# NVIDIA-Merlin/HugeCTR

Hardware: AMD Instinct MI355X
Metric: samples/sec (whole node) + embedding-gather HBM GB/s, DLRM Criteo-1TB (higher is better)
Workload: dtype fp16; 1 GPU; BASELINE configs[2]: DLRM Criteo-1TB slot_size_array, LocalizedSlotSparseEmbeddingHash, emb_dim=128, SGD, bs=65536 per GPU (weak scaling); batch_per_gpu=65536, global_batch=65536, slots=26, emb_dim=128, table_rows_total=187767399, parallelism=slot-sharded x1 + dp1, exchange=none (1 GPU), gather_fused_into_interaction=True

## Files before the change

### hugectr_amd/_lib.py

```python
import ctypes
import os

import torch
from ctypes import (POINTER, Structure, c_char_p, c_float, c_int, c_int64, c_size_t,
                    c_uint64, c_void_p)

_HERE = os.path.dirname(os.path.abspath(__file__))
_VARIANT = os.environ.get("HCTR_LIB_VARIANT", "")
LIB_PATH = os.path.join(_HERE, f"libhugectr_amd{'_' + _VARIANT if _VARIANT else ''}.so")

OPT_FTRL, OPT_ADAM, OPT_RMSPROP, OPT_ADAGRAD, OPT_NESTEROV, OPT_MOMENTUM_SGD, OPT_SGD = range(7)
UPDATE_LOCAL, UPDATE_GLOBAL, UPDATE_LAZY_GLOBAL = range(3)
EMB_DISTRIBUTED, EMB_LOCALIZED = 0, 1
KEY_U32, KEY_I64 = 0, 1
F32, F16, BF16 = 0, 1, 2


class EmbeddingParams(Structure):
    _fields_ = [
        ("embedding_type", c_int), ("key_type", c_int), ("out_dtype", c_int),
        ("train_batch_size", c_size_t), ("evaluate_batch_size", c_size_t),
        ("max_vocabulary_size_per_gpu", c_size_t), ("embedding_vec_size", c_size_t),
        ("max_feature_num", c_size_t), ("slot_num", c_size_t), ("combiner", c_int),
        ("slot_size_array", POINTER(c_size_t)),
# ... 44 lines not shown
    "hctr_ht_value_head": (c_int, [_P, _P, POINTER(c_size_t)]),
    "hctr_ht_set_value_head": (c_int, [_P, c_size_t, _P]),
    "hctr_ht_table_size": (c_size_t, [_P]),
    "hctr_ht_dump": (c_int, [_P, _P, _P, POINTER(c_size_t), _P]),
    "hctr_ht_error_flags": (c_int, [_P, _P, POINTER(ctypes.c_uint32)]),
    "hctr_ht_recover": (c_int, [_P, _P, c_size_t, _P]),
    "hctr_forward_pool": (c_int, [c_size_t, c_int, c_int, _P, c_int, _P, _P, _P, c_int, _P]),
    "hctr_forward_pool_weighted": (c_int, [c_size_t, c_int, c_int, _P, _P, _P, _P, _P, _P]),
    "hctr_expand_key_grads": (c_int, [c_size_t, c_int, c_int, _P, _P, _P, _P, _P]),
    "hctr_forward_pool_multihot": (c_int, [c_size_t, c_int, c_int, _P, c_int, _P, _P, _P, c_int, _P]),
    "hctr_forward_pool_mapped": (c_int, [c_size_t, c_int, c_int, _P, c_int, _P, _P, _P, c_int, c_int,
                                         c_size_t, c_size_t, _P, _P]),
    "hctr_ebc_route_whole": (c_int, [c_size_t, c_int, _P, _P, _P, c_int, _P, _P, _P, _P, c_size_t,
                                     _P]),
    "hctr_forward_reorder": (c_int, [c_size_t, c_int, c_int, c_int, _P, _P, c_int, _P]),
    "hctr_backward_reorder": (c_int, [c_size_t, c_int, c_int, c_int, _P, _P, c_int, _P]),
    "hctr_emb_create": (c_int, [POINTER(EmbeddingParams), POINTER(_P)]),
    "hctr_emb_destroy": (c_int, [_P]),
    "hctr_emb_init_params": (c_int, [_P, _P]),
    "hctr_emb_forward": (c_int, [_P, c_int, _P, _P, c_size_t, _P, _P]),
    "hctr_emb_forward_scale": (c_int, [_P, c_int, _P, _P]),
    "hctr_emb_poll_overflow": (c_int, [_P, _P]),
    "hctr_emb_backward": (c_int, [_P, _P, _P]),
    "hctr_emb_get_wgrad": (c_int, [_P, _P, _P]),
    "hctr_emb_update_params": (c_int, [_P, _P]),
    "hctr_emb_set_learning_rate": (c_int, [_P, c_float]),
    "hctr_emb_get_vocabulary_size": (c_int, [_P, _P, POINTER(c_size_t)]),
    "hctr_emb_get_max_vocabulary_size": (c_size_t, [_P]),
    "hctr_emb_slots_on_rank": (c_size_t, [_P]),
    "hctr_emb_check_overflow": (c_int, [_P, _P]),
    "hctr_emb_dump": (c_int, [_P, _P, _P, _P, POINTER(c_size_t), _P]),
    "hctr_emb_load": (c_int, [_P, _P, _P, _P, c_size_t, _P]),
    "hctr_emb_table_ptr": (_P, [_P]),
    "hctr_emb_opt_state_ptr": (_P, [_P, c_int]),
    "hctr_emb_value_index_ptr": (_P, [_P]),
    "hctr_emb_reset": (c_int, [_P, _P]),
    "hctr_emb_profiling": (c_int, [_P, c_int]),
    "hctr_emb_profile_get": (c_int, [_P, c_int, POINTER(ctypes.c_double), POINTER(c_uint64)]),
    "hctr_ebc_keys_to_indices": (c_int, [_P, c_int, c_size_t, c_int64, c_int, _P, _P]),
    "hctr_ebc_route_workspace_bytes": (c_size_t, [c_size_t, c_int]),
    "hctr_ebc_route_keys": (c_int, [c_size_t, c_int, c_int, _P, _P, _P, _P, c_int, _P, _P, _P, _P, _P]),
    "hctr_ebc_bucket_counts": (c_int, [c_size_t, c_int, c_int, c_int, _P, c_int, _P, _P]),
    "hctr_ebc_network_forward": (c_int, [c_size_t, c_int, c_int, c_int, _P, _P, _P, c_int, _P, _P, c_int, _P]),
    "hctr_ebc_network_backward": (c_int, [c_size_t, c_int, c_int, c_int, _P, _P, _P, c_int, _P, _P, c_int, _P]),
    "hctr_updater_create": (c_int, [c_size_t, c_size_t, c_int, POINTER(_P)]),
    "hctr_updater_destroy": (c_int, [_P]),
    "hctr_updater_update": (c_int, [_P, c_size_t, c_size_t, _P, _P, _P, c_int, c_int, c_int, c_float,
                                    c_float, c_float, c_float, c_float, c_float, c_uint64, _P, _P,
                                    _P, _P]),
    "hctr_interaction_fwd": (c_int, [c_size_t, c_int, c_int, _P, _P, _P, c_int, _P]),
    "hctr_interaction_bwd": (c_int, [c_size_t, c_int, c_int, _P, _P, _P, _P, _P, c_int, _P]),
    "hctr_cross_v1_fwd": (c_int, [c_size_t, c_int, c_int, _P, _P, _P, _P, _P, _P]),
    "hctr_cross_v1_bwd": (c_int, [c_size_t, c_int, c_int, _P, _P, _P, _P, _P, _P, _P, _P, _P, _P]),
    "hctr_cross_v1_bwd_workspace_bytes": (c_size_t, [c_size_t, c_int, c_int]),
    "hctr_det_create": (c_int, [c_size_t, _SZP, c_char_p, c_size_t, c_int, c_uint64, POINTER(_P)]),
    "hctr_det_destroy": (c_int, [_P]),
    "hctr_det_num_classes": (c_size_t, [_P]),
    "hctr_det_lookup": (c_int, [_P, _P, _P, c_size_t, _SZP, _SZP, c_size_t, _P]),
    "hctr_det_lookup_unsafe": (c_int, [_P, _P, _P, c_size_t, _SZP, _SZP, c_size_t, _P]),
    "hctr_det_scatter_add": (c_int, [_P, _P, _P, c_size_t, _SZP, _SZP, c_size_t, _P]),
    "hctr_det_scatter_update": (c_int, [_P, _P, _P, c_size_t, _SZP, _SZP, c_size_t, _P]),
    "hctr_det_remove": (c_int, [_P, _P, c_size_t, _SZP, _SZP, c_size_t, _P]),
    "hctr_det_export": (c_int, [_P, c_size_t, _P, _P, c_size_t, _SZP, _P]),
    "hctr_det_lookup_index": (c_int, [_P, c_size_t, _P, c_size_t, c_int, _P, _P]),
    "hctr_det_rows": (c_int, [_P, c_size_t, POINTER(_P), _SZP]),
    "hctr_det_row_store": (c_int, [_P, POINTER(_P), POINTER(ctypes.c_uint64)]),
    "hctr_det_state_store": (c_int, [_P, c_int, POINTER(_P), POINTER(_P), _P]),
    "hctr_det_lookup_rows": (c_int, [_P, _P, c_size_t, _SZP, _SZP, c_size_t, c_int, _P, _P,
                                     POINTER(c_uint64), _P]),
    "hctr_radix_sort_temp_bytes": (c_size_t, [c_size_t]),
    "hctr_radix_sort_pairs_u32": (c_int, [_P, c_size_t, _P, _P, _P, _P, c_size_t, c_int, _P]),
    "hctr_static_lookup": (c_int, [_P, c_int, c_size_t, _P, c_size_t, _P, _P, c_size_t, _P, _P, _P,
                                   _P, _P, _P, _P]),
    "hctr_forward_pool_ptrs": (c_int, [c_size_t, c_int, c_int, _P, _P, _P, c_int, _P]),
    "hctr_forward_pool_ptrs_mapped": (c_int, [c_size_t, c_int, c_int, _P, _P, _P, c_int, c_size_t,
                                              c_size_t, _P]),
    "hctr_ebc_routed_keys_to_indices": (c_int, [c_size_t, c_int, c_int, _P, _P, _P, _P, _P]),
    "hctr_ebc_local_reduce": (c_int, [_P, c_size_t, c_size_t, _P, _P, c_uint64, _P, _P, c_int, _SZP,
                                      _P, _P, _P, _P]),
    "hctr_det_clear": (c_int, [_P, _P]),
    "hctr_det_size_per_class": (c_int, [_P, _SZP, _P]),
    "hctr_det_capacity_per_class": (c_int, [_P, _SZP]),
    "hctr_det_repair_count": (c_int, [_P, POINTER(ctypes.c_uint64)]),
    "hctr_det_update": (c_int, [_P, _P, POINTER(DetOptParams), _P, c_size_t, _SZP, _SZP, c_size_t,
                                _P, _P, _P]),
    "hctr_cache_create": (c_int, [c_size_t, c_int, c_int, POINTER(_P)]),
    "hctr_cache_destroy": (c_int, [_P]),
    "hctr_cache_capacity_in_set": (c_size_t, [_P]),
    "hctr_cache_query": (c_int, [_P, _P, c_size_t, _P, _P, _P, _P, _P]),
    "hctr_cache_replace": (c_int, [_P, _P, c_size_t, _P, _P]),
    "hctr_cache_update": (c_int, [_P, _P, c_size_t, _P, _P]),
    "hctr_cache_dump": (c_int, [_P, _P, _P, c_size_t, c_size_t, _P]),
    "hctr_tiered_create": (c_int, [c_size_t, c_int, c_size_t, POINTER(_P)]),
    "hctr_tiered_destroy": (c_int, [_P]),
    "hctr_tiered_host_rows": (_P, [_P]),
    "hctr_tiered_cache": (_P, [_P]),
    "hctr_tiered_lookup": (c_int, [_P, _P, c_size_t, _P, _P, _P]),
    "hctr_tiered_scatter": (c_int, [_P, _P, c_size_t, _P, c_int, c_float, _P]),
    "hctr_tiered_flush": (c_int, [_P, _P]),
    "hctr_uvm_create": (c_int, [c_size_t, c_size_t, c_size_t, c_int, c_float, c_int, POINTER(_P)]),
    "hctr_uvm_destroy": (c_int, [_P]),
    "hctr_uvm_tier": (_P, [_P]),
    "hctr_uvm_add": (c_int, [_P, _P, _P, c_size_t]),
    "hctr_uvm_query": (c_int, [_P, _P, c_size_t, _P, _P]),
    "hctr_uvm_clear": (c_int, [_P, _P]),
    "hctr_uvm_lookup": (c_int, [_P, _P, c_size_t, _P, _P, _P, _P]),
    "hctr_uvm_scatter_rows": (c_int, [_P, _P, c_size_t, _P, c_int, c_float, _P]),
    "hctr_uvm_check_overflow": (c_int, [_P, _P]),
    "hctr_uvm_size": (c_int, [_P, _P, POINTER(c_size_t)]),
    "hctr_uniq_create": (c_int, [c_size_t, POINTER(_P)]),
    "hctr_uniq_destroy": (c_int, [_P]),
    "hctr_uniq_plan": (c_int, [_P, c_size_t, c_size_t, c_int, c_int, c_int, c_int, c_int, _P,
                               c_uint64, _P, _P, _P, _P]),
    "hctr_uniq_gather_rows": (c_int, [c_size_t, c_int, _P, _P, _P, c_int, _P]),
    "hctr_uniq_expand": (c_int, [c_size_t, c_int, _P, _P, _P, _P, c_int, c_int, _P, _P, _P, _P, _P]),
    "hctr_ebc_uniq_plan_workspace_bytes": (c_size_t, [c_size_t]),
    "hctr_ebc_uniq_plan": (c_int, [c_size_t, c_int, c_size_t, _P, _P, c_uint64, _P, _P, _P, _P,
                                   c_size_t, _P]),
    "hctr_ebc_uniq_gather_rows": (c_int, [c_size_t, c_int, _P, _P, c_uint64, _P, c_int, _P]),
    "hctr_ebc_uniq_network_forward": (c_int, [c_size_t, c_int, c_int, c_int, _P, _P, _P, c_int, _P,
                                              _P, _P, _P, _P, _P, _P, c_int, _P]),
    "hctr_ebc_uniq_backward_workspace_bytes": (c_size_t, [c_size_t, c_size_t, c_int, c_int]),
    "hctr_ebc_uniq_network_backward": (c_int, [_P, c_size_t, c_int, c_int, c_int, _P, _P, _P, _P,
                                               c_int, c_int, _P, _P, _P, c_size_t, c_size_t, _P,
                                               c_int, _P, _P, c_size_t, _P]),
    "hctr_interaction_fwd_indexed": (c_int, [c_size_t, c_int, c_int, _P, _P, _P, _P, c_int, _P]),
    "hctr_ebc_scale_average": (c_int, [c_size_t, c_int, c_int, _P, _P, c_int, _P, c_int, c_int, _P]),
    "hctr_interaction_fwd_gather": (c_int, [c_size_t, c_int, c_int, _P, _P, _P, _P, _P, c_int, _P]),
    "hctr_emb_forward_interaction": (c_int, [_P, c_int, _P, _P, _P, _P]),
    "hctr_interaction_bwd_gather": (c_int, [c_size_t, c_int, c_int, _P, _P, _P, _P, _P, _P, c_int,
                                            _P]),
    "hctr_emb_backward_interaction": (c_int, [_P, _P, _P, _P, _P, _P]),
    "hctr_interaction_bwd_indexed": (c_int, [c_size_t, c_int, c_int, _P, _P, _P, _P, _P, _P, c_int,
                                             _P]),
    "hctr_interaction_bwd_indexed_scatter": (c_int, [c_size_t, c_int, c_int, _P, _P, _P, _P, _P, _P,
                                                     c_int, _P]),
    "hctr_updater_set_ftrl": (c_int, [_P, c_float, c_float, c_float]),
    "hctr_updater_set_grad_map": (c_int, [_P, c_size_t, c_size_t]),
    "hctr_updater_set_row_bound": (c_int, [_P, ctypes.c_uint64]),
    "hctr_updater_reduce_presorted": (c_int, [_P, c_size_t, c_size_t, _P, _P, _P, _P, c_int,
                                              c_size_t, _P, _P]),
    "hctr_emb_index": (c_int, [_P, c_int, _P, _P, c_size_t, _P]),
    "hctr_emb_index_ahead": (c_int, [_P, _P, _P, c_size_t, _P]),
    "hctr_emb_index_adopt": (c_int, [_P]),
    "hctr_emb_update_rows": (c_int, [_P, c_size_t, _P, _P, _P, c_int, _P]),
    "hctr_relu_bwd_bias_workspace_bytes": (c_size_t, [c_size_t, c_int]),
    "hctr_relu_bwd_bias": (c_int, [c_size_t, c_int, _P, _P, _P, _P, _P, c_int, _P]),
    "hctr_logit_head_workspace_bytes": (c_size_t, [c_int]),
    "hctr_logit_head": (c_int, [c_size_t, c_int, _P, _P, _P, _P, c_float, _P, _P, _P, _P, _P, c_int,
                                _P]),
    "hctr_skinny_fc_fwd": (c_int, [c_size_t, c_int, c_int, _P, _P, _P, _P, c_int, _P]),
    "hctr_skinny_fc_bwd_workspace_bytes": (c_size_t, [c_int]),
    "hctr_skinny_fc_bwd": (c_int, [c_size_t, c_int, c_int, _P, _P, _P, _P, _P, _P, c_int, _P]),
    "hctr_sum_groups": (c_int, [c_int, c_size_t, _P, c_int, _P, _P]),
    "hctr_sgd_shadow": (c_int, [c_size_t, c_float, c_float, _P, _P, _P, c_int, _P]),
    "hctr_bce_loss_workspace_bytes": (c_size_t, []),
    "hctr_bce_loss": (c_int, [c_size_t, _P, _P, c_float, _P, _P, _P, c_int, _P]),
    "hctr_convert_transpose16": (c_int, [c_size_t, c_int, c_int, _P, _P, _P, c_int, _P]),
    "hctr_gemm_nt16": (c_int, [c_size_t, c_int, c_int, _P, c_int, _P, c_int, _P, c_int, c_int, _P, _P,
                               _P, _P, c_int, _P]),
    "hctr_cross_v2_bwd_step_workspace_bytes": (c_size_t, [c_size_t, c_int]),
    "hctr_cross_v2_bwd_step": (c_int, [c_size_t, c_int, _P, _P, _P, _P, _P, _P, _P, c_int, c_int, _P]),
    "hctr_lru_create": (c_int, [c_size_t, c_size_t, c_int, c_int, c_char_p, c_uint64, POINTER(_P)]),
    "hctr_lru_destroy": (c_int, [_P]),
    "hctr_lru_lookup_index": (c_int, [_P, _P, c_size_t, c_int, _P, _P, _P, _SZP, _P]),
    "hctr_lru_find": (c_int, [_P, _P, c_size_t, _P, _P]),
    "hctr_lru_rows": (c_int, [_P, POINTER(_P), _SZP]),
    "hctr_lru_state": (c_int, [_P, c_int, POINTER(_P), _P]),
    "hctr_lru_export": (c_int, [_P, _P, _P, _P, _P, c_size_t, _SZP, _P]),
    "hctr_lru_size": (c_int, [_P, _SZP, _P]),
    "hctr_lru_rejected_count": (c_int, [_P, POINTER(c_uint64), _P]),
    "hctr_lru_capacity": (c_int, [_P, _SZP, _SZP]),
    "hctr_lru_lookup_index_filtered": (c_int, [_P, _P, c_size_t, c_uint64, _P, _P, _P, _SZP, _P]),
    "hctr_lru_filtered_count": (c_int, [_P, POINTER(c_uint64), _P]),
    "hctr_lru_compact": (c_int, [_P, c_size_t, c_size_t, _P, _P, _P, _P, _P, _P, _P, _P, _SZP,
                                 _P]),
    "hctr_lru_export_if": (c_int, [_P, c_uint64, _P, _P, _P, _P, c_size_t, _SZP, _SZP, _P]),
    "hctr_lru_create_tiered": (c_int, [c_size_t, c_size_t, c_int, c_int, c_char_p, c_uint64,
                                       c_size_t, POINTER(_P)]),
    "hctr_lru_create_growing": (c_int, [c_size_t, c_size_t, c_float, c_size_t, c_int, c_int,
                                        c_char_p, c_uint64, c_size_t, POINTER(_P)]),
    "hctr_lru_growth": (c_int, [_P, _SZP, _SZP, POINTER(c_uint64)]),
    "hctr_lru_placement": (c_int, [_P, _SZP, _SZP, _SZP]),
    "hctr_lru_host_part": (c_int, [_P, c_int, POINTER(_P)]),
    "hctr_lru_gather_slots": (c_int, [_P, c_int, _P, c_size_t, _P, _P]),
    "hctr_lru_scatter_slots": (c_int, [_P, c_int, _P, c_size_t, _P, c_int, _P]),
    "hctr_lru_apply_update": (c_int, [_P, _P, c_size_t, c_size_t, _P, _P, _P, c_int, c_int,
                                      c_float, c_float, c_float, c_float, c_float, c_float,
                                      c_uint64, _P]),
    "hctr_dist_select": (c_int, [_P, c_int, c_size_t, c_int, _P, _P, _P, _P, c_size_t, _P]),
    "hctr_indexed_row_copy": (c_int, [POINTER(RowCopyTask), c_int, c_int, c_int, _P]),
    "hctr_ebc_io_create": (c_int, [c_size_t, c_int, c_int, POINTER(_P)]),
    "hctr_ebc_io_destroy": (c_int, [_P]),
    "hctr_ebc_io_chunk": (c_int, [_P, c_int, POINTER(_P), POINTER(_P), POINTER(_P), POINTER(_P)]),
    "hctr_ebc_io_wait": (c_int, [_P, c_int]),
    "hctr_ebc_io_check": (c_int, [_P, c_int, c_size_t, c_int, c_int, c_uint64, _P, _P]),
    "hctr_ebc_io_import_static": (c_int, [_P, c_int, c_size_t, c_int, c_int, c_uint64, c_uint64, _P,
                                          _P, _P, _P]),
    "hctr_ebc_io_select": (c_int, [_P, c_int, c_size_t, c_int, c_int, c_uint64, _P, _P, _P, _P, _SZP,
                                   _P]),
    "hctr_ebc_io_scatter_rows": (c_int, [c_size_t, c_int, _P, _P, _P, c_uint64, _P]),
    "hctr_ebc_io_export_static": (c_int, [_P, c_int, c_size_t, c_uint64, c_uint64, _P, _P, _P, _P]),
    "hctr_ebc_group_segments": (c_int, [c_size_t, c_size_t, _P, _P, _P, c_size_t, _P, _P]),
    "hctr_ebc_hybrid_row_ptrs": (c_int, [c_size_t, c_size_t, _P, _P, _P, c_int, _P, c_int, _P,
                                         c_size_t, _P, _P, _P]),
    "hctr_ebc_hybrid_key_grads": (c_int, [c_size_t, c_int, _P, _P, c_size_t, _P, c_int, c_size_t,
                                          c_size_t, _P, _P]),
    "hctr_metric_accumulate_temp_bytes": (c_size_t, []),
    "hctr_metric_accumulate": (c_int, [_P, c_int, _P, c_size_t, c_int, _P, _P, c_size_t, c_size_t,
                                       _P, _P, c_size_t, _P]),
    "hctr_metric_auc_temp_bytes": (c_size_t, [c_size_t]),
    "hctr_metric_auc": (c_int, [_P, c_size_t, _P, _P, c_size_t, _P, _P]),
    "hctr_metric_ndcg_temp_bytes": (c_size_t, [c_size_t]),
    "hctr_metric_ndcg": (c_int, [_P, c_size_t, _P, _P, c_size_t, _P, _P]),
}
METRIC_MAX_CLASSES = 256
METRIC_COUNTER_WORDS = 264

EXPORTED_SYMBOLS = tuple(_SIGNATURES.keys())


class HugeCTRAmdError(RuntimeError):
    """The reference surfaces C++ exceptions as Python RuntimeError; so do we."""


def _load():
    if not os.path.exists(LIB_PATH):
        raise ImportError(
            f"{LIB_PATH} not found: build it with `python -c 'import __graft_entry__ as g; "
            "g.build()'` (hipcc --offload-arch=gfx950). There is no CPU fallback.")
    lib = ctypes.CDLL(LIB_PATH)
    for name, (res, args) in _SIGNATURES.items():
        fn = getattr(lib, name)
        fn.restype = res
        fn.argtypes = args
    return lib


lib = _load()


def last_error() -> str:
    msg = lib.hctr_last_error()
    return msg.decode() if msg else ""


def check(rc: int) -> None:
    if rc != 0:
        raise HugeCTRAmdError(f"hugectr_amd error {rc}: {last_error()}")


def ptr(t):
    if t is None:
        return None
    return c_void_p(t.data_ptr())


def stream_ptr():
    import torch
    return c_void_p(torch.cuda.current_stream().cuda_stream)
```

### hugectr_amd/csrc/dense_ops.hip

```cpp
#include "block_prims.h"
#include "common.h"
#include "cvt16.h"

namespace hctr {
namespace {

typedef float f32x4 __attribute__((ext_vector_type(4)));
typedef unsigned int u32x4 __attribute__((ext_vector_type(4)));

constexpr int kBlock = 256;
constexpr int kWavesPerBlock = kBlock / 64;

__device__ __forceinline__ float wave_sum(float v) {
#pragma unroll
  for (int d = 32; d >= 1; d >>= 1) v += __shfl_xor(v, d, 64);
  return v;
}

template <int NPL>
__global__ void __launch_bounds__(kBlock)
    cross_v1_fwd_kernel(size_t batch, int w, int layers, const float* __restrict__ x0,
                        const float* __restrict__ kernels, const float* __restrict__ biases,
                        float* __restrict__ outputs, float* __restrict__ hiddens) {
  const int lane = threadIdx.x & 63;
// ... 135 lines not shown
  __shared__ float red[kBlock * 8];
  const int n8 = n / 8;
  const int c8 = threadIdx.x % cw, g = threadIdx.x / cw;
  const bool live = g < rg;
  const size_t r0 = (size_t)blockIdx.x * kRbRows;
  const size_t r1 = r0 + kRbRows < rows ? r0 + kRbRows : rows;
  for (int cc = c8; cc - c8 < n8; cc += cw) {
    float acc[8] = {0.f, 0.f, 0.f, 0.f, 0.f, 0.f, 0.f, 0.f};
    if (live && cc < n8) {
#pragma unroll 4
      for (size_t r = r0 + g; r < r1; r += rg) {
        const u32x4 gv = *reinterpret_cast<const u32x4*>(dy + r * n + cc * 8);
        const u32x4 av = *reinterpret_cast<const u32x4*>(y + r * n + cc * 8);
        u32x4 o;
#pragma unroll
        for (int e = 0; e < 4; e++) {
          const unsigned short g0 = (unsigned short)(gv[e] & 0xFFFFu);
          const unsigned short g1 = (unsigned short)(gv[e] >> 16);
          const float y0 = H::to_f32((unsigned short)(av[e] & 0xFFFFu));
          const float y1 = H::to_f32((unsigned short)(av[e] >> 16));
          const unsigned short z0 = y0 > 0.f ? g0 : (unsigned short)0;
          const unsigned short z1 = y1 > 0.f ? g1 : (unsigned short)0;
          acc[2 * e] += H::to_f32(z0);
          acc[2 * e + 1] += H::to_f32(z1);
          o[e] = (unsigned)z0 | ((unsigned)z1 << 16);
        }
        *reinterpret_cast<u32x4*>(dz + r * n + cc * 8) = o;
      }
    }
#pragma unroll
    for (int e = 0; e < 8; e++) red[e * kBlock + threadIdx.x] = acc[e];
    __syncthreads();
    if (g == 0 && cc < n8) {
      float* p = partial + (size_t)blockIdx.x * n + cc * 8;
#pragma unroll
      for (int e = 0; e < 8; e++) {
        float sum = 0.f;
        for (int k = 0; k < rg; k++) sum += red[e * kBlock + k * cw + c8];
        p[e] = sum;
      }
    }
    __syncthreads();
  }
}

template <bool BF, bool FIRST>
__global__ void __launch_bounds__(kBlock)
    cross_v2_bwd_step_kernel(size_t rows, int n, int cw, int rg, int rpt,
                             const unsigned short* __restrict__ dy,
                             const unsigned short* __restrict__ x0,
                             const unsigned short* __restrict__ hm, unsigned short* __restrict__ acc_io,
                             unsigned short* __restrict__ s0, float* __restrict__ partial) {
  using H = H16<BF>;
  __shared__ float red[kBlock * 8];
  const int n8 = n / 8;
  const int c8 = threadIdx.x % cw, g = threadIdx.x / cw;
  const bool live = g < rg;
  const size_t r0 = (size_t)blockIdx.x * (size_t)rpt;
  const size_t r1 = r0 + (size_t)rpt < rows ? r0 + (size_t)rpt : rows;
  const int cc = (int)blockIdx.y * cw + c8;
  {
    float sum[8] = {0.f, 0.f, 0.f, 0.f, 0.f, 0.f, 0.f, 0.f};
    if (live && cc < n8) {
#pragma unroll 4
      for (size_t r = r0 + g; r < r1; r += rg) {
        const size_t at = r * n + cc * 8;
        const u32x4 gv = *reinterpret_cast<const u32x4*>(dy + at);
        const u32x4 xv = *reinterpret_cast<const u32x4*>(x0 + at);
        const u32x4 hv = *reinterpret_cast<const u32x4*>(hm + at);
        u32x4 av = {0u, 0u, 0u, 0u};
        if (!FIRST) av = *reinterpret_cast<const u32x4*>(acc_io + at);
        u32x4 so, ao;
#pragma unroll
        for (int e = 0; e < 4; e++) {
          const float g0 = H::to_f32((unsigned short)(gv[e] & 0xFFFFu));
          const float g1 = H::to_f32((unsigned short)(gv[e] >> 16));
          const unsigned short p0 = H::from_f32(g0 * H::to_f32((unsigned short)(xv[e] & 0xFFFFu)));
          const unsigned short p1 = H::from_f32(g1 * H::to_f32((unsigned short)(xv[e] >> 16)));
          sum[2 * e] += H::to_f32(p0);
          sum[2 * e + 1] += H::to_f32(p1);
          so[e] = (unsigned)p0 | ((unsigned)p1 << 16);
          float a0 = g0 * H::to_f32((unsigned short)(hv[e] & 0xFFFFu));
          float a1 = g1 * H::to_f32((unsigned short)(hv[e] >> 16));
          if (!FIRST) {
            a0 += H::to_f32((unsigned short)(av[e] & 0xFFFFu));
            a1 += H::to_f32((unsigned short)(av[e] >> 16));
          }
          ao[e] = (unsigned)H::from_f32(a0) | ((unsigned)H::from_f32(a1) << 16);
        }
        *reinterpret_cast<u32x4*>(s0 + at) = so;
        *reinterpret_cast<u32x4*>(acc_io + at) = ao;
      }
    }
#pragma unroll
    for (int e = 0; e < 8; e++) red[e * kBlock + threadIdx.x] = sum[e];
    __syncthreads();
    if (g == 0 && cc < n8) {
      float* p = partial + (size_t)blockIdx.x * n + cc * 8;
#pragma unroll
      for (int e = 0; e < 8; e++) {
        float t = 0.f;
        for (int k = 0; k < rg; k++) t += red[e * kBlock + k * cw + c8];
        p[e] = t;
      }
    }
    __syncthreads();
  }
}

__global__ void __launch_bounds__(kBlock)
    colsum_partials_kernel(size_t tiles, int n, const float* __restrict__ partial,
                           float* __restrict__ db) {
  __shared__ f32x4 red[kBlock];
  const int c4 = blockIdx.x * 8 + (threadIdx.x & 7), tg = threadIdx.x >> 3;
  const bool live = c4 * 4 < n;
  f32x4 s = {0.f, 0.f, 0.f, 0.f};
  if (live) {
#pragma unroll 8
    for (size_t t = tg; t < tiles; t += 32)
      s += *reinterpret_cast<const f32x4*>(partial + t * n + c4 * 4);
  }
  red[threadIdx.x] = s;
  __syncthreads();
  if (tg == 0 && live) {
    f32x4 sum = {0.f, 0.f, 0.f, 0.f};
#pragma unroll
    for (int k = 0; k < 32; k++) sum += red[k * 8 + threadIdx.x];
    *reinterpret_cast<f32x4*>(db + c4 * 4) = sum;
  }
}

template <bool BF>
__global__ void __launch_bounds__(kBlock)
    sum_groups_kernel(int groups, size_t n8, const unsigned short* __restrict__ in,
                      float* __restrict__ out) {
  using H = H16<BF>;
  const size_t i = (size_t)blockIdx.x * kBlock + threadIdx.x;
  if (i >= n8) return;
  float acc[8] = {0.f, 0.f, 0.f, 0.f, 0.f, 0.f, 0.f, 0.f};
#pragma unroll 4
  for (int g = 0; g < groups; g++) {
    const u32x4 v = *reinterpret_cast<const u32x4*>(in + ((size_t)g * n8 + i) * 8);
#pragma unroll
    for (int e = 0; e < 4; e++) {
      acc[2 * e] += H::to_f32((unsigned short)(v[e] & 0xFFFFu));
      acc[2 * e + 1] += H::to_f32((unsigned short)(v[e] >> 16));
    }
  }
  f32x4* o = reinterpret_cast<f32x4*>(out + i * 8);
  o[0] = f32x4{acc[0], acc[1], acc[2], acc[3]};
  o[1] = f32x4{acc[4], acc[5], acc[6], acc[7]};
}

template <bool BF>
__global__ void __launch_bounds__(kBlock)
    sgd_shadow_kernel(size_t n4, float lr, float grad_scale, float* __restrict__ w,
                      const float* __restrict__ g, unsigned short* __restrict__ w16) {
  using H = H16<BF>;
  for (size_t i = (size_t)blockIdx.x * kBlock + threadIdx.x; i < n4;
       i += (size_t)gridDim.x * kBlock) {
    f32x4 wv = reinterpret_cast<f32x4*>(w)[i];
    const f32x4 gv = reinterpret_cast<const f32x4*>(g)[i];
    wv -= lr * grad_scale * gv;
    reinterpret_cast<f32x4*>(w)[i] = wv;
    const unsigned lo = (unsigned)H::from_f32(wv[0]) | ((unsigned)H::from_f32(wv[1]) << 16);
    const unsigned hi = (unsigned)H::from_f32(wv[2]) | ((unsigned)H::from_f32(wv[3]) << 16);
    reinterpret_cast<uint2*>(w16)[i] = make_uint2(lo, hi);
  }
}

constexpr int kBceBlocks = 256;

template <typename T>
__global__ void __launch_bounds__(kBlock)
    bce_kernel(size_t batch, const T* __restrict__ logit, const float* __restrict__ label,
               float grad_scale, T* __restrict__ dlogit, float* __restrict__ partial) {
  __shared__ float smem[kBlock / 64];
  float val = 0.f;
  for (size_t i = (size_t)blockIdx.x * kBlock + threadIdx.x; i < batch;
       i += (size_t)gridDim.x * kBlock) {
    const float x = ld_as_f32(logit + i);
    const float y = label[i];
    float g;
    if (x >= 0.f) {
      const float e = expf(-x);
      g = (1.f - y) - e / (1.f + e);
      val += x * (1.f - y) + logf(1.f + e);
    } else {
      const float e = expf(x);
      g = -y + e / (1.f + e);
      val += -x * y + logf(1.f + e);
    }
    if (dlogit) st_from_f32(dlogit + i, g * grad_scale);
  }
  const float tot = block_reduce_sum<float, kBlock>(val, smem);
  if (threadIdx.x == 0) partial[blockIdx.x] = tot;
}

__global__ void __launch_bounds__(kBlock)
    bce_finish_kernel(int blocks, size_t batch, const float* __restrict__ partial,
                      float* __restrict__ loss) {
  __shared__ float smem[kBlock / 64];
  const float v = (int)threadIdx.x < blocks ? partial[threadIdx.x] : 0.f;
  const float tot = block_reduce_sum<float, kBlock>(v, smem);
  if (threadIdx.x == 0) *loss = tot / (float)batch;
}

constexpr int kHeadBlocks = 1024;
constexpr int kHeadMaxSeg = 8;

template <typename T, int NSEG, int ROWS>
__global__ void __launch_bounds__(kBlock)
    logit_head_kernel(size_t batch, int K, const T* __restrict__ x, const T* __restrict__ w,
                      const T* __restrict__ bias, const float* __restrict__ label,
                      float grad_scale, T* __restrict__ dx, float* __restrict__ partial) {
  HCTR_DYN_LDS(float, lds);
  const int lane = threadIdx.x & 63, wv = threadIdx.x >> 6;
  const float4 zero4 = make_float4(0.f, 0.f, 0.f, 0.f);
  float4 wr[NSEG], acc[NSEG];
#pragma unroll
  for (int j = 0; j < NSEG; j++) {
    const int k = j * 256 + lane * 4;
    wr[j] = k < K ? ld4_as_f32<T>(w + k) : zero4;
    acc[j] = zero4;
  }
  const float b0 = ld_as_f32(bias);
  float db = 0.f, loss = 0.f;
  const size_t nw = (size_t)gridDim.x * (kBlock / 64);
  for (size_t r0 = ((size_t)blockIdx.x * (kBlock / 64) + wv) * ROWS; r0 < batch; r0 += nw * ROWS) {
    float4 xv[ROWS][NSEG];
    float dot[ROWS];
#pragma unroll
    for (int i = 0; i < ROWS; i++) {
      const size_t r = r0 + i;
      dot[i] = 0.f;
#pragma unroll
      for (int j = 0; j < NSEG; j++) {
        const int k = j * 256 + lane * 4;
        xv[i][j] = (r < batch && k < K) ? ld4_as_f32<T>(x + r * (size_t)K + k) : zero4;
        dot[i] += xv[i][j].x * wr[j].x + xv[i][j].y * wr[j].y + xv[i][j].z * wr[j].z +
                  xv[i][j].w * wr[j].w;
      }
    }
#pragma unroll
    for (int o = 32; o > 0; o >>= 1)
#pragma unroll
      for (int i = 0; i < ROWS; i++) dot[i] += __shfl_xor(dot[i], o);
#pragma unroll
    for (int i = 0; i < ROWS; i++) {
      const size_t r = r0 + i;
      if (r >= batch) break;
      const float z = dot[i] + b0;
      const float y = label[r];
      float g, l;
      if (z >= 0.f) {
        const float e = expf(-z);
        g = (1.f - y) - e / (1.f + e);
        l = z * (1.f - y) + logf(1.f + e);
      } else {
        const float e = expf(z);
        g = -y + e / (1.f + e);
        l = -z * y + logf(1.f + e);
      }
      const float dz = g * grad_scale;
      loss += l;
      db += dz;
#pragma unroll
      for (int j = 0; j < NSEG; j++) {
        const int k = j * 256 + lane * 4;
        if (k < K) {
          acc[j].x += dz * xv[i][j].x;
          acc[j].y += dz * xv[i][j].y;
          acc[j].z += dz * xv[i][j].z;
          acc[j].w += dz * xv[i][j].w;
          if (dx)
            st4_from_f32<T>(dx + r * (size_t)K + k, make_float4(dz * wr[j].x, dz * wr[j].y,
                                                                 dz * wr[j].z, dz * wr[j].w));
        }
      }
    }
  }
  float* mine = lds + wv * (K + 2);
#pragma unroll
  for (int j = 0; j < NSEG; j++) {
    const int k = j * 256 + lane * 4;
    if (k < K) {
      mine[k] = acc[j].x;
      mine[k + 1] = acc[j].y;
      mine[k + 2] = acc[j].z;
      mine[k + 3] = acc[j].w;
    }
  }
  if (lane == 0) {
    mine[K] = db;
    mine[K + 1] = loss;
  }
  __syncthreads();
  float* out = partial + (size_t)blockIdx.x * (K + 2);
  for (int k = threadIdx.x; k < K + 2; k += kBlock) {
    float t = 0.f;
    for (int q = 0; q < kBlock / 64; q++) t += lds[q * (K + 2) + k];
    out[k] = t;
  }
}

__global__ void __launch_bounds__(1024)
    logit_head_finish_kernel(int blocks, int K, size_t batch, const float* __restrict__ partial,
                             float* __restrict__ dw, float* __restrict__ db,
                             float* __restrict__ loss) {
  __shared__ float part[16][64];
  const int c = threadIdx.x & 63, grp = threadIdx.x >> 6;
  const int k = blockIdx.x * 64 + c;
  const int chunk = (blocks + 15) / 16;
  const int b0 = grp * chunk, b1 = min(blocks, b0 + chunk);
  float t = 0.f;
  if (k < K + 2) {
// ... 130 lines not shown
    }
#pragma unroll
    for (int u = 0; u < kSkinnyUnroll; u++) {
      if (r0 + (size_t)u * step < batch) {
        const float4 gf = cvt4_as_f32<T>(g[u]), af = cvt4_as_f32<T>(a[u]);
        const float d[4] = {af.x > 0.f ? gf.x : 0.f, af.y > 0.f ? gf.y : 0.f,
                            af.z > 0.f ? gf.z : 0.f, af.w > 0.f ? gf.w : 0.f};
        const float xr = lane < K ? round16<T>(xl[u]) : 0.f;
#pragma unroll
        for (int j = 0; j < 4; j++) dbv[j] += d[j];
#pragma unroll
        for (int k = 0; k < kSkinnyK; k += 2) {
          const v2f xk = v2f{__shfl(xr, k), __shfl(xr, k + 1)};
#pragma unroll
          for (int j = 0; j < 4; j++) acc[j][k / 2] += xk * d[j];
        }
      }
    }
#pragma unroll
    for (int u = 0; u < kSkinnyUnroll; u++) {
      g[u] = gn[u];
      a[u] = an[u];
      xl[u] = xn[u];
    }
  }
  const int stride = kSkinnyK + 1;
  for (int q = 0; q < kRows; q++) {
    if (sub == q && live) {
#pragma unroll
      for (int j = 0; j < 4; j++) {
        float* d = lds + (size_t)(n0 + j) * stride;
#pragma unroll
        for (int k = 0; k < kSkinnyK; k++) {
          const float v = (k & 1) ? acc[j][k / 2].y : acc[j][k / 2].x;
          d[k] = (q == 0 ? 0.f : d[k]) + v;
        }
        d[kSkinnyK] = (q == 0 ? 0.f : d[kSkinnyK]) + dbv[j];
      }
    }
    __syncthreads();
  }
  float* out = partial + (size_t)blockIdx.x * N * stride;
  for (int i = threadIdx.x; i < N * stride; i += kSkinnyBwdBlock) out[i] = lds[i];
}

typedef float v4f __attribute__((ext_vector_type(4)));
constexpr int kMfmaUnroll = 4;

template <typename T>
__global__ void __launch_bounds__(kSkinnyBwdBlock)
    skinny_fc_bwd_mfma_kernel(size_t batch, int K, int N, const float* __restrict__ x,
                              const T* __restrict__ dy, const T* __restrict__ y,
                              float* __restrict__ partial) {
  HCTR_DYN_LDS(float, lds);
  const int lane = threadIdx.x & 63;
  const int wv = __builtin_amdgcn_readfirstlane(threadIdx.x >> 6);
  constexpr int kWaves = kSkinnyBwdBlock / 64;
  const int ngroups = (N + 127) / 128;
  const int rsets = kWaves / ngroups;
  const int ng = wv % ngroups, rs = wv / ngroups;
  const bool active = rs < rsets;
  const int c = lane & 15, ri = lane >> 4;
  const int n0 = ng * 128 + 8 * c;
  const bool has_n = n0 < N;
  const int n0c = has_n ? n0 : 0;
  const int kc = c < K ? c : K - 1;
  v4f acc[8];
#pragma unroll
  for (int t = 0; t < 8; t++) acc[t] = v4f{0.f, 0.f, 0.f, 0.f};
  const size_t last = batch - 1;
  const size_t step = (size_t)gridDim.x * rsets;
  if (active) {
    for (size_t g16 = (size_t)blockIdx.x * rsets + rs; g16 * 16 < batch; g16 += step) {
      uint4 gq[kMfmaUnroll], aq[kMfmaUnroll];
      float xv[kMfmaUnroll];
#pragma unroll
      for (int u = 0; u < kMfmaUnroll; u++) {
        const size_t r = min(g16 * 16 + u * 4 + ri, last);
        gq[u] = *reinterpret_cast<const uint4*>(dy + r * (size_t)N + n0c);
        aq[u] = *reinterpret_cast<const uint4*>(y + r * (size_t)N + n0c);
        xv[u] = x[r * (size_t)K + kc];
      }
#pragma unroll
      for (int u = 0; u < kMfmaUnroll; u++) {
        const bool ok = has_n && g16 * 16 + u * 4 + ri < batch;
        const float4 g0 = cvt4_as_f32<T>(make_uint2(gq[u].x, gq[u].y));
        const float4 g1 = cvt4_as_f32<T>(make_uint2(gq[u].z, gq[u].w));
        const float4 a0 = cvt4_as_f32<T>(make_uint2(aq[u].x, aq[u].y));
        const float4 a1 = cvt4_as_f32<T>(make_uint2(aq[u].z, aq[u].w));
        const float d[8] = {(ok && a0.x > 0.f) ? g0.x : 0.f, (ok && a0.y > 0.f) ? g0.y : 0.f,
                            (ok && a0.z > 0.f) ? g0.z : 0.f, (ok && a0.w > 0.f) ? g0.w : 0.f,
                            (ok && a1.x > 0.f) ? g1.x : 0.f, (ok && a1.y > 0.f) ? g1.y : 0.f,
                            (ok && a1.z > 0.f) ? g1.z : 0.f, (ok && a1.w > 0.f) ? g1.w : 0.f};
        const float b = c < K ? round16<T>(xv[u]) : (c == K ? 1.f : 0.f);
#pragma unroll
        for (int t = 0; t < 8; t++)
          acc[t] = __builtin_amdgcn_mfma_f32_16x16x4f32(d[t], b, acc[t], 0, 0, 0);
      }
    }
  }
  const int stride = kSkinnyK + 1;
  const int col = c == K ? kSkinnyK : c;
  for (int q = 0; q < rsets; q++) {
    if (active && rs == q && c <= K) {
#pragma unroll
      for (int t = 0; t < 8; t++) {
#pragma unroll
        for (int reg = 0; reg < 4; reg++) {
          const int n = ng * 128 + 8 * (4 * ri + reg) + t;
          if (n < N) {
            float* d = lds + (size_t)n * stride + col;
            *d = (q == 0 ? 0.f : *d) + acc[t][reg];
          }
        }
      }
    }
    __syncthreads();
  }
  float* out = partial + (size_t)blockIdx.x * N * stride;
  for (int i = threadIdx.x; i < N * stride; i += kSkinnyBwdBlock) out[i] = lds[i];
}

__global__ void __launch_bounds__(1024)
    skinny_fc_finish_kernel(int blocks, int K, int N, const float* __restrict__ partial,
                            float* __restrict__ dw, float* __restrict__ db) {
  __shared__ float part[16][64];
  const int stride = kSkinnyK + 1;
  const int total = N * stride;
  const int c = threadIdx.x & 63, grp = threadIdx.x >> 6;
  const int i = blockIdx.x * 64 + c;
  const int chunk = (blocks + 15) / 16;
  const int b0 = grp * chunk, b1 = min(blocks, b0 + chunk);
  float t = 0.f;
  if (i < total) {
    int b = b0;
    for (; b + 8 <= b1; b += 8) {
      float v[8];
#pragma unroll
      for (int u = 0; u < 8; u++) v[u] = partial[(size_t)(b + u) * total + i];
#pragma unroll
      for (int u = 0; u < 8; u++) t += v[u];
    }
    for (; b < b1; b++) t += partial[(size_t)b * total + i];
  }
  part[grp][c] = t;
  __syncthreads();
  if (grp == 0 && i < total) {
    float tot = 0.f;
#pragma unroll
    for (int q = 0; q < 16; q++) tot += part[q][c];
    const int n = i / stride, k = i % stride;
    if (k == kSkinnyK) db[n] = tot;
    else if (k < K) dw[(size_t)n * K + k] = tot;
  }
}

constexpr int kCrossBwdWaves = 256 * 4;

}
}

using namespace hctr;

extern "C" {

#define HCTR_CROSS_DISPATCH(MACRO)       \
  if (npl <= 1) MACRO(1)                 \
  else if (npl <= 2) MACRO(2)            \
  else if (npl <= 4) MACRO(4)            \
  else if (npl <= 8) MACRO(8)            \
  else if (npl <= 16) MACRO(16)          \
  else if (npl <= 32) MACRO(32)          \
  else MACRO(64)

int hctr_cross_v1_fwd(size_t batch, int width, int layers, const float* x0, const float* kernels,
                      const float* biases, float* outputs, float* hiddens, hctr_stream_t stream) {
  HCTR_REQUIRE(width >= 1 && layers >= 1, "shape");
  HCTR_REQUIRE(width <= 64 * 64, "cross v1: width > 4096 not supported");
  if (batch == 0) return HCTR_OK;
  HCTR_REQUIRE(x0 && kernels && biases && outputs && hiddens, "null pointer");
  hipStream_t s = as_stream(stream);
  const int npl = (width + 63) / 64;
  const int grid = grid_for(batch * 64, kBlock);
#define HCTR_CF(N_)                                                                            \
  hipLaunchKernelGGL(cross_v1_fwd_kernel<N_>, dim3(grid), dim3(kBlock), 0, s, batch, width,    \
                     layers, x0, kernels, biases, outputs, hiddens);
  HCTR_CROSS_DISPATCH(HCTR_CF)
#undef HCTR_CF
  HCTR_LAUNCH_CHECK();
  return HCTR_OK;
}

size_t hctr_cross_v1_bwd_workspace_bytes(size_t batch, int width, int layers) {
  (void)batch;
  return (size_t)kCrossBwdWaves * layers * 2 * width * sizeof(float);
}

int hctr_cross_v1_bwd(size_t batch, int width, int layers, const float* x0, const float* kernels,
                      const float* outputs, const float* hiddens, const float* out_grad,
                      float* in_grad, float* kernel_grads, float* bias_grads, float* workspace,
                      hctr_stream_t stream) {
  HCTR_REQUIRE(width >= 1 && layers >= 1, "shape");
  HCTR_REQUIRE(width <= 64 * 64, "cross v1: width > 4096 not supported");
  HCTR_REQUIRE(x0 && kernels && outputs && hiddens && out_grad && in_grad && kernel_grads &&
                   bias_grads && workspace,
               "null pointer");
  hipStream_t s = as_stream(stream);
  const int npl = (width + 63) / 64;
  const int grid = kCrossBwdWaves / kWavesPerBlock;
  const size_t lds_bytes = (size_t)layers * 2 * width * sizeof(float);
  if (lds_bytes <= 60 * 1024) {
#define HCTR_CB(N_)                                                                           \
  hipLaunchKernelGGL((cross_v1_bwd_kernel<N_, true>), dim3(kCrossBwdWaves), dim3(64), lds_bytes, \
                     s, batch, width, layers, x0, kernels, outputs, hiddens, out_grad, in_grad,  \
                     workspace);
    HCTR_CROSS_DISPATCH(HCTR_CB)
#undef HCTR_CB
  } else {
#define HCTR_CB(N_)                                                                           \
  hipLaunchKernelGGL((cross_v1_bwd_kernel<N_, false>), dim3(grid), dim3(kBlock), 0, s, batch, \
                     width, layers, x0, kernels, outputs, hiddens, out_grad, in_grad, workspace);
    HCTR_CROSS_DISPATCH(HCTR_CB)
#undef HCTR_CB
  }
  HCTR_LAUNCH_CHECK();
  hipLaunchKernelGGL(cross_v1_reduce_kernel,
                     dim3((unsigned)ceil_div<size_t>((size_t)layers * 2 * width, 32)),
                     dim3(kBlock), 0, s, (size_t)kCrossBwdWaves, width, layers, workspace,
                     kernel_grads, bias_grads);
  HCTR_LAUNCH_CHECK();
  return HCTR_OK;
}

size_t hctr_relu_bwd_bias_workspace_bytes(size_t rows, int n) {
  return ceil_div<size_t>(rows, (size_t)kRbRows) * (size_t)n * sizeof(float);
}

int hctr_relu_bwd_bias(size_t rows, int n, const void* dy, const void* y, void* dz, float* db,
                       float* workspace, int dtype, hctr_stream_t stream) {
  HCTR_REQUIRE(n > 0 && n % 8 == 0, "n must be a multiple of 8");
  HCTR_REQUIRE(dtype == HCTR_EMB_BF16 || dtype == HCTR_EMB_F16, "16-bit dtypes only");
  if (rows == 0) return HCTR_OK;
  HCTR_REQUIRE(dy && y && dz && db && workspace, "null pointer");
  hipStream_t s = as_stream(stream);
  const size_t tiles = ceil_div<size_t>(rows, (size_t)kRbRows);
  const int cw = n / 8 < kBlock ? n / 8 : kBlock;
  const int rg = kBlock / cw;
  if (dtype == HCTR_EMB_BF16)
    hipLaunchKernelGGL(relu_bwd_bias_kernel<true>, dim3((unsigned)tiles), dim3(kBlock), 0, s, rows,
                       n, cw, rg, (const unsigned short*)dy, (const unsigned short*)y,
                       (unsigned short*)dz, workspace);
  else
    hipLaunchKernelGGL(relu_bwd_bias_kernel<false>, dim3((unsigned)tiles), dim3(kBlock), 0, s,
                       rows, n, cw, rg, (const unsigned short*)dy, (const unsigned short*)y,
                       (unsigned short*)dz, workspace);
  HCTR_LAUNCH_CHECK();
  hipLaunchKernelGGL(colsum_partials_kernel, dim3(ceil_div<int>(n, 32)), dim3(kBlock), 0, s,
                     tiles, n, workspace, db);
  HCTR_LAUNCH_CHECK();
  return HCTR_OK;
}

size_t hctr_cross_v2_bwd_step_workspace_bytes(size_t batch, int width) {
  if (batch == 0 || width <= 0) return 0;
  return ceil_div<size_t>(batch, (size_t)cross_step_rows_per_tile(batch, width)) * (size_t)width *
         sizeof(float);
}

int hctr_cross_v2_bwd_step(size_t batch, int width, const void* dy, const void* x0, const void* h,
                           void* acc, void* s0, float* db, float* workspace, int first, int dtype,
                           hctr_stream_t stream) {
  HCTR_REQUIRE(width > 0 && width % 8 == 0, "width must be a multiple of 8");
  HCTR_REQUIRE(dtype == HCTR_EMB_BF16 || dtype == HCTR_EMB_F16, "16-bit dtypes only");
  if (batch == 0) return HCTR_OK;
  HCTR_REQUIRE(dy && x0 && h && acc && s0 && db && workspace, "null pointer");
  hipStream_t s = as_stream(stream);
  const int cw = width / 8 < kBlock ? width / 8 : kBlock;
  const int rg = kBlock / cw;
  const int rpt = cross_step_rows_per_tile(batch, width);
  const size_t tiles = ceil_div<size_t>(batch, (size_t)rpt);
  const unsigned col_blocks = (unsigned)ceil_div<int>(width / 8, cw);
#define HCTR_CROSS_STEP(BF_, FIRST_)                                                              \
  hipLaunchKernelGGL((cross_v2_bwd_step_kernel<BF_, FIRST_>), dim3((unsigned)tiles, col_blocks),   \
                     dim3(kBlock), 0, s, batch, width, cw, rg, rpt, (const unsigned short*)dy,     \
                     (const unsigned short*)x0, (const unsigned short*)h, (unsigned short*)acc,    \
                     (unsigned short*)s0, workspace)
  if (dtype == HCTR_EMB_BF16) {
    if (first) HCTR_CROSS_STEP(true, true);
    else HCTR_CROSS_STEP(true, false);
  } else {
    if (first) HCTR_CROSS_STEP(false, true);
    else HCTR_CROSS_STEP(false, false);
  }
#undef HCTR_CROSS_STEP
  HCTR_LAUNCH_CHECK();
  hipLaunchKernelGGL(colsum_partials_kernel, dim3(ceil_div<int>(width, 32)), dim3(kBlock), 0, s,
                     tiles, width, workspace, db);
  HCTR_LAUNCH_CHECK();
  return HCTR_OK;
}

int hctr_sum_groups(int groups, size_t n, const void* in, int dtype, float* out,
                    hctr_stream_t stream) {
  HCTR_REQUIRE(groups > 0 && n % 8 == 0, "n must be a multiple of 8");
  HCTR_REQUIRE(dtype == HCTR_EMB_BF16 || dtype == HCTR_EMB_F16, "16-bit dtypes only");
  if (n == 0) return HCTR_OK;
  HCTR_REQUIRE(in && out, "null pointer");
  hipStream_t s = as_stream(stream);
  const size_t n8 = n / 8;
  const dim3 grid((unsigned)ceil_div<size_t>(n8, (size_t)kBlock));
  if (dtype == HCTR_EMB_BF16)
    hipLaunchKernelGGL(sum_groups_kernel<true>, grid, dim3(kBlock), 0, s, groups, n8,
                       (const unsigned short*)in, out);
  else
    hipLaunchKernelGGL(sum_groups_kernel<false>, grid, dim3(kBlock), 0, s, groups, n8,
                       (const unsigned short*)in, out);
  HCTR_LAUNCH_CHECK();
  return HCTR_OK;
}

int hctr_sgd_shadow(size_t n, float lr, float grad_scale, float* w, const float* g, void* w16,
                    int dtype, hctr_stream_t stream) {
  HCTR_REQUIRE(n % 4 == 0, "n must be a multiple of 4");
  HCTR_REQUIRE(dtype == HCTR_EMB_BF16 || dtype == HCTR_EMB_F16, "16-bit shadow dtypes only");
  if (n == 0) return HCTR_OK;
  HCTR_REQUIRE(w && g && w16, "null pointer");
  hipStream_t s = as_stream(stream);
  const dim3 grid(grid_for(n / 4, kBlock, 4096));
  if (dtype == HCTR_EMB_BF16)
    hipLaunchKernelGGL(sgd_shadow_kernel<true>, grid, dim3(kBlock), 0, s, n / 4, lr, grad_scale, w,
                       g, (unsigned short*)w16);
  else
    hipLaunchKernelGGL(sgd_shadow_kernel<false>, grid, dim3(kBlock), 0, s, n / 4, lr, grad_scale,
                       w, g, (unsigned short*)w16);
  HCTR_LAUNCH_CHECK();
  return HCTR_OK;
}

size_t hctr_bce_loss_workspace_bytes(void) { return kBceBlocks * sizeof(float); }

int hctr_bce_loss(size_t batch, const void* logit, const float* label, float grad_scale,
                  void* dlogit, float* loss, float* workspace, int dtype, hctr_stream_t stream) {
  HCTR_REQUIRE(batch > 0, "empty batch");
  HCTR_REQUIRE(logit && label && loss && workspace, "null pointer");
  hipStream_t s = as_stream(stream);
  const int blocks = (int)(ceil_div<size_t>(batch, (size_t)kBlock) < (size_t)kBceBlocks
                               ? ceil_div<size_t>(batch, (size_t)kBlock)
                               : (size_t)kBceBlocks);
  switch (dtype) {
    case HCTR_EMB_F32:
      hipLaunchKernelGGL(bce_kernel<float>, dim3(blocks), dim3(kBlock), 0, s, batch,
                         (const float*)logit, label, grad_scale, (float*)dlogit, workspace);
      break;
    case HCTR_EMB_F16:
      hipLaunchKernelGGL(bce_kernel<__half>, dim3(blocks), dim3(kBlock), 0, s, batch,
                         (const __half*)logit, label, grad_scale, (__half*)dlogit, workspace);
      break;
    case HCTR_EMB_BF16:
      hipLaunchKernelGGL(bce_kernel<__hip_bfloat16>, dim3(blocks), dim3(kBlock), 0, s, batch,
                         (const __hip_bfloat16*)logit, label, grad_scale, (__hip_bfloat16*)dlogit,
                         workspace);
      break;
    default:
      HCTR_REQUIRE(false, "bad dtype");
  }
  HCTR_LAUNCH_CHECK();
  hipLaunchKernelGGL(bce_finish_kernel, dim3(1), dim3(kBlock), 0, s, blocks, batch, workspace, loss);
  HCTR_LAUNCH_CHECK();
  return HCTR_OK;
}

size_t hctr_logit_head_workspace_bytes(int k) { return (size_t)kHeadBlocks * (k + 2) * sizeof(float); }

int hctr_logit_head(size_t batch, int k, const void* x, const void* w, const void* bias,
                    const float* label, float grad_scale, void* dx, float* dw, float* db,
                    float* loss, float* workspace, int dtype, hctr_stream_t stream) {
  HCTR_REQUIRE(batch > 0 && k >= 4 && k % 4 == 0 && k <= 256 * kHeadMaxSeg,
               "logit head: K must be a multiple of 4 and <= 2048");
  HCTR_REQUIRE(dtype == HCTR_EMB_F16 || dtype == HCTR_EMB_BF16, "16-bit activations");
  HCTR_REQUIRE(x && w && bias && label && dw && db && loss && workspace, "null pointer");
  HCTR_REQUIRE(reinterpret_cast<uintptr_t>(x) % 8 == 0 && reinterpret_cast<uintptr_t>(w) % 8 == 0 &&
                   (dx == nullptr || reinterpret_cast<uintptr_t>(dx) % 8 == 0),
               "8-byte aligned buffers");
  hipStream_t s = as_stream(stream);
  const int nseg = (k + 255) / 256;
  const int rows = nseg <= 1 ? 8 : (nseg <= 2 ? 4 : (nseg <= 4 ? 2 : 1));
  const int blocks = (int)std::min<size_t>(
      (size_t)kHeadBlocks, ceil_div<size_t>(batch, (size_t)(kBlock / 64) * rows));
  const size_t lds = (size_t)(kBlock / 64) * (k + 2) * sizeof(float);
#define HCTR_HEAD(T_, NSEG_, ROWS_)                                                               \
  hipLaunchKernelGGL((logit_head_kernel<T_, NSEG_, ROWS_>), dim3(blocks), dim3(kBlock), lds, s,   \
                     batch, k, (const T_*)x, (const T_*)w, (const T_*)bias, label, grad_scale,    \
                     (T_*)dx, workspace)
#define HCTR_HEAD_T(T_)                       \
  if (nseg <= 1) HCTR_HEAD(T_, 1, 8);         \
  else if (nseg <= 2) HCTR_HEAD(T_, 2, 4);    \
  else if (nseg <= 4) HCTR_HEAD(T_, 4, 2);    \
  else HCTR_HEAD(T_, 8, 1);
  if (dtype == HCTR_EMB_BF16) {
    HCTR_HEAD_T(__hip_bfloat16)
  } else {
    HCTR_HEAD_T(__half)
  }
#undef HCTR_HEAD_T
#undef HCTR_HEAD
  HCTR_LAUNCH_CHECK();
  hipLaunchKernelGGL(logit_head_finish_kernel, dim3(ceil_div<int>(k + 2, 64)), dim3(1024), 0, s,
                     blocks, k, batch, workspace, dw, db, loss);
  HCTR_LAUNCH_CHECK();
  return HCTR_OK;
}

static int skinny_check(size_t batch, int k, int n, int dtype) {
  HCTR_REQUIRE(batch > 0 && k >= 1 && k <= kSkinnyK, "skinny fc: 1 <= K <= 16");
  HCTR_REQUIRE(n >= 4 && n % 4 == 0 && n <= 512, "skinny fc: N a multiple of 4, <= 512");
  HCTR_REQUIRE(dtype == HCTR_EMB_F16 || dtype == HCTR_EMB_BF16, "16-bit weights / activations");
  return HCTR_OK;
}

int hctr_skinny_fc_fwd(size_t batch, int k, int n, const float* x, const void* w, const void* bias,
                       void* y, int dtype, hctr_stream_t stream) {
  HCTR_TRY(skinny_check(batch, k, n, dtype));
  HCTR_REQUIRE(x && w && bias && y, "null pointer");
  HCTR_REQUIRE(reinterpret_cast<uintptr_t>(y) % 8 == 0, "8-byte aligned output");
  hipStream_t s = as_stream(stream);
  size_t rows = ceil_div<size_t>(batch, 1024);
  rows = std::min<size_t>(256, (rows + 1) / 2 * 2);
  const int blocks = (int)ceil_div<size_t>(batch, rows);
  const size_t lds = rows * kSkinnyK * sizeof(float);
  if (dtype == HCTR_EMB_BF16)
    hipLaunchKernelGGL(skinny_fc_fwd_kernel<__hip_bfloat16>, dim3(blocks), dim3(kBlock), lds, s,
                       batch, k, n, (int)rows, x, (const __hip_bfloat16*)w,
                       (const __hip_bfloat16*)bias, (__hip_bfloat16*)y);
  else
    hipLaunchKernelGGL(skinny_fc_fwd_kernel<__half>, dim3(blocks), dim3(kBlock), lds, s, batch, k, n,
                       (int)rows, x, (const __half*)w, (const __half*)bias, (__half*)y);
  HCTR_LAUNCH_CHECK();
  return HCTR_OK;
}

size_t hctr_skinny_fc_bwd_workspace_bytes(int n) {
  return (size_t)kSkinnyBlocks * n * (kSkinnyK + 1) * sizeof(float);
}

int hctr_skinny_fc_bwd(size_t batch, int k, int n, const float* x, const void* dy, const void* y,
                       float* dw, float* db, float* workspace, int dtype, hctr_stream_t stream) {
  HCTR_TRY(skinny_check(batch, k, n, dtype));
  HCTR_REQUIRE(x && dy && y && dw && db && workspace, "null pointer");
  HCTR_REQUIRE(reinterpret_cast<uintptr_t>(dy) % 8 == 0 && reinterpret_cast<uintptr_t>(y) % 8 == 0,
               "8-byte aligned activations");
  hipStream_t s = as_stream(stream);
  const size_t lds = (size_t)n * (kSkinnyK + 1) * sizeof(float);
  const char* mode = getenv("HCTR_SKINNY_BWD");
  const bool want_mfma = mode ? strcmp(mode, "valu") != 0 : kSkinnyBwdMfmaDefault;
  if (want_mfma && k < kSkinnyK && n % 8 == 0 && reinterpret_cast<uintptr_t>(dy) % 16 == 0 &&
      reinterpret_cast<uintptr_t>(y) % 16 == 0) {
    const int rsets = (kSkinnyBwdBlock / 64) / ceil_div<int>(n, 128);
    const int blocks = (int)std::min<size_t>((size_t)kSkinnyBlocks,
                                             ceil_div<size_t>(batch, (size_t)rsets * 16));
    if (dtype == HCTR_EMB_BF16)
      hipLaunchKernelGGL(skinny_fc_bwd_mfma_kernel<__hip_bfloat16>, dim3(blocks),
                         dim3(kSkinnyBwdBlock), lds, s, batch, k, n, x, (const __hip_bfloat16*)dy,
                         (const __hip_bfloat16*)y, workspace);
    else
      hipLaunchKernelGGL(skinny_fc_bwd_mfma_kernel<__half>, dim3(blocks), dim3(kSkinnyBwdBlock), lds,
                         s, batch, k, n, x, (const __half*)dy, (const __half*)y, workspace);
    HCTR_LAUNCH_CHECK();
    hipLaunchKernelGGL(skinny_fc_finish_kernel, dim3(ceil_div<int>(n * (kSkinnyK + 1), 64)),
                       dim3(1024), 0, s, blocks, k, n, workspace, dw, db);
    HCTR_LAUNCH_CHECK();
    return HCTR_OK;
  }
  const int blocks = (int)std::min<size_t>(
      (size_t)kSkinnyBlocks, ceil_div<size_t>(batch, kSkinnyBwdBlock / kSkinnyLanes));
  if (dtype == HCTR_EMB_BF16)
    hipLaunchKernelGGL(skinny_fc_bwd_kernel<__hip_bfloat16>, dim3(blocks), dim3(kSkinnyBwdBlock), lds, s,
                       batch, k, n, x, (const __hip_bfloat16*)dy, (const __hip_bfloat16*)y,
                       workspace);
  else
    hipLaunchKernelGGL(skinny_fc_bwd_kernel<__half>, dim3(blocks), dim3(kSkinnyBwdBlock), lds, s, batch, k, n,
                       x, (const __half*)dy, (const __half*)y, workspace);
  HCTR_LAUNCH_CHECK();
  hipLaunchKernelGGL(skinny_fc_finish_kernel, dim3(ceil_div<int>(n * (kSkinnyK + 1), 64)),
                     dim3(1024), 0, s, blocks, k, n, workspace, dw, db);
  HCTR_LAUNCH_CHECK();
  return HCTR_OK;
}

}
```

### hugectr_amd/dense.py

```python
from __future__ import annotations

import os

from typing import List, Sequence

import torch

from ._lib import check, lib, ptr, stream_ptr

_DT16 = {torch.float16: 1, torch.bfloat16: 2}
_DT = {torch.float32: 0, torch.float16: 1, torch.bfloat16: 2}


def split_k_wgrad(dy: torch.Tensor, x: torch.Tensor, groups: int = 16,
                  out: torch.Tensor = None) -> torch.Tensor:
    B, o = dy.shape
    i = x.shape[1]
    g = groups
    while g > 1 and B % g != 0:
        g //= 2
    if g <= 1 or min(o, i) < 8:
        r = dy.t() @ x
        if out is not None:
            out.copy_(r)
            return out
        return r
    p = torch.bmm(dy.view(g, B // g, o).transpose(1, 2), x.view(g, B // g, i))
    if p.is_cuda and p.dtype in _DT16 and (o * i) % 8 == 0:
        if out is None:
            out = torch.empty((o, i), dtype=torch.float32, device=p.device)
        check(lib.hctr_sum_groups(g, o * i, ptr(p), _DT16[p.dtype], ptr(out), stream_ptr()))
        return out
    r = p.float().sum(0)
    if out is not None:
        out.copy_(r)
        return out
    return r


def bce_with_logits(logit: torch.Tensor, label: torch.Tensor, grad_scale: float):
    x = logit.detach().contiguous()
    y = label.contiguous()
    assert x.is_cuda and y.dtype == torch.float32 and x.numel() == y.numel()
    dlogit = torch.empty_like(x)
    loss = torch.empty(1, dtype=torch.float32, device=x.device)
    ws = torch.empty(lib.hctr_bce_loss_workspace_bytes() // 4, dtype=torch.float32, device=x.device)
    check(lib.hctr_bce_loss(x.numel(), ptr(x), ptr(y), float(grad_scale), ptr(dlogit), ptr(loss),
                            ptr(ws), _DT[x.dtype], stream_ptr()))
    return loss, dlogit


class _LinearFn(torch.autograd.Function):

    @staticmethod
    def forward(ctx, x, w_master, b_master, w16, b16, relu: bool, groups: int, gw=None, gb=None):
        x = x.contiguous()
        ctx.gw, ctx.gb = gw, gb
        if relu:
            y = torch._addmm_activation(b16, x, w16.t(), use_gelu=False)
        else:
            y = torch.addmm(b16, x, w16.t())
        ctx.relu, ctx.groups = relu, groups
        ctx.save_for_backward(x, w16, y if relu else None)
        return y

    @staticmethod
    def backward(ctx, dy):
        x, w16, y = ctx.saved_tensors
        dy = dy.contiguous()
        n = dy.shape[1]
        if ctx.relu and n % 8 == 0 and dy.dtype in _DT16 and dy.is_cuda:
            dz = torch.empty_like(dy)
            db = ctx.gb if ctx.gb is not None else torch.empty(n, dtype=torch.float32,
                                                             device=dy.device)
            ws = torch.empty(lib.hctr_relu_bwd_bias_workspace_bytes(dy.shape[0], n) // 4,
                             dtype=torch.float32, device=dy.device)
            check(lib.hctr_relu_bwd_bias(dy.shape[0], n, ptr(dy), ptr(y), ptr(dz), ptr(db), ptr(ws),
                                         _DT16[dy.dtype], stream_ptr()))
            dy = dz
        else:
            if ctx.relu:
                dy = torch.ops.aten.threshold_backward(dy, y, 0)
            db = dy.sum(0, dtype=torch.float32)
            if ctx.gb is not None:
                ctx.gb.copy_(db)
        dx = dy @ w16 if ctx.needs_input_grad[0] else None
        dw = split_k_wgrad(dy, x, ctx.groups, out=ctx.gw)
        if ctx.gw is not None:
            return dx, None, None, None, None, None, None, None, None
        return dx, dw.float(), db, None, None, None, None, None, None


class _SkinnyFirstFn(torch.autograd.Function):

    @staticmethod
    def forward(ctx, x, w_master, b_master, w16, b16, gw=None, gb=None):
        x = x.contiguous()
        B, K = x.shape
        N = w16.shape[0]
        if os.environ.get("HCTR_SKINNY_FC_FWD", "gemm") == "hip":
            y = torch.empty((B, N), dtype=w16.dtype, device=x.device)
            check(lib.hctr_skinny_fc_fwd(B, K, N, ptr(x), ptr(w16), ptr(b16), ptr(y),
                                         _DT16[w16.dtype], stream_ptr()))
        else:
            y = torch._addmm_activation(b16, x.to(w16.dtype), w16.t(), use_gelu=False)
        ctx.gw, ctx.gb = gw, gb
        ctx.save_for_backward(x, y)
        return y

    @staticmethod
    def backward(ctx, dy):
        x, y = ctx.saved_tensors
        dy = dy.contiguous()
        B, K = x.shape
        N = y.shape[1]
        dev = x.device
        dw = ctx.gw if ctx.gw is not None else torch.empty((N, K), dtype=torch.float32, device=dev)
        db = ctx.gb if ctx.gb is not None else torch.empty(N, dtype=torch.float32, device=dev)
        ws = torch.empty(lib.hctr_skinny_fc_bwd_workspace_bytes(N) // 4, dtype=torch.float32,
                         device=dev)
        check(lib.hctr_skinny_fc_bwd(B, K, N, ptr(x), ptr(dy), ptr(y), ptr(dw), ptr(db), ptr(ws),
                                     _DT16[y.dtype], stream_ptr()))
        if ctx.gw is not None:
            return None, None, None, None, None, None, None
        return None, dw, db, None, None, None, None


class _LogitHeadFn(torch.autograd.Function):

    @staticmethod
    def forward(ctx, x, w_master, b_master, w16, b16, label, grad_scale: float, gw=None, gb=None):
        x = x.contiguous()
        B, K = x.shape
        dev = x.device
        dx = torch.empty_like(x) if ctx.needs_input_grad[0] else None
        dw = gw if gw is not None else torch.empty((1, K), dtype=torch.float32, device=dev)
        db = gb if gb is not None else torch.empty(1, dtype=torch.float32, device=dev)
        loss = torch.empty(1, dtype=torch.float32, device=dev)
        ws = torch.empty(lib.hctr_logit_head_workspace_bytes(K) // 4, dtype=torch.float32, device=dev)
        label = label.contiguous()
        check(lib.hctr_logit_head(B, K, ptr(x), ptr(w16), ptr(b16), ptr(label),
                                  float(grad_scale), ptr(dx), ptr(dw), ptr(db), ptr(loss), ptr(ws),
                                  _DT16[x.dtype], stream_ptr()))
        ctx.flat = gw is not None
        ctx.dx = dx
        ctx.dw, ctx.db = (None, None) if ctx.flat else (dw, db)
        return loss

    @staticmethod
    def backward(ctx, _grad_loss):
        dx, dw, db = ctx.dx, ctx.dw, ctx.db
        ctx.dx = ctx.dw = ctx.db = None
        return dx, dw, db, None, None, None, None, None, None


class FusedMLP(torch.nn.Module):

    def __init__(self, dims: Sequence[int], last_relu: bool, dtype=torch.bfloat16,
                 wgrad_groups: int = 16):
        super().__init__()
        self.dims = list(dims)
        self.dtype = dtype
        self.wgrad_groups = wgrad_groups
        self.relu = [True] * (len(dims) - 2) + [last_relu]
        self.weights = torch.nn.ParameterList()
        self.biases = torch.nn.ParameterList()
        for i in range(len(dims) - 1):
            lin = torch.nn.Linear(dims[i], dims[i + 1])
            self.weights.append(torch.nn.Parameter(lin.weight.detach().clone()))
            self.biases.append(torch.nn.Parameter(lin.bias.detach().clone()))
        self._w16: List[torch.Tensor] = []
        self._b16: List[torch.Tensor] = []
        self.flat_w = self.flat_g = self.flat_w16 = None
        self._gw: List[torch.Tensor] = []
        self._gb: List[torch.Tensor] = []

    def flatten(self):
        dev = self.weights[0].device
        sizes = [p.numel() for p in list(self.weights) + list(self.biases)]
        offs, tot = [], 0
        for n in sizes:
            offs.append(tot)
            tot += (n + 3) // 4 * 4
        self.flat_w = torch.zeros(tot, dtype=torch.float32, device=dev)
        self.flat_g = torch.zeros(tot, dtype=torch.float32, device=dev)
        self.flat_w16 = torch.zeros(tot, dtype=self.dtype, device=dev)
        params = list(self.weights) + list(self.biases)
        views16 = []
        self._gw, self._gb = [], []
        for p, o, n in zip(params, offs, sizes):
            v = self.flat_w[o:o + n].view_as(p)
            v.copy_(p.data)
            p.data = v
            views16.append(self.flat_w16[o:o + n].view_as(p))
        nl = len(self.weights)
        self._w16, self._b16 = views16[:nl], views16[nl:]
        gviews = [self.flat_g[o:o + n].view_as(p) for p, o, n in zip(params, offs, sizes)]
        self._gw, self._gb = gviews[:nl], gviews[nl:]
        self.flat_w16.copy_(self.flat_w)
        return self

    def sgd_step(self, lr: float, grad_scale: float = 1.0):
        check(lib.hctr_sgd_shadow(self.flat_w.numel(), float(lr), float(grad_scale),
                                  ptr(self.flat_w), ptr(self.flat_g), ptr(self.flat_w16),
                                  _DT16[self.dtype], stream_ptr()))

    def refresh_shadow(self):
        if self.flat_w is not None:
            self.flat_w16.copy_(self.flat_w)
            return
        if not self._w16:
            self._w16 = [w.detach().to(self.dtype) for w in self.weights]
            self._b16 = [b.detach().to(self.dtype) for b in self.biases]
        else:
            torch._foreach_copy_(self._w16 + self._b16,
                                 [w.detach() for w in self.weights] +
                                 [b.detach() for b in self.biases])

    def _skinny_first(self, x) -> bool:
        return (self.relu[0] and self.dims[0] <= 16 and self.dims[1] % 4 == 0 and
                self.dims[1] <= 512 and self.dtype in _DT16 and x.is_cuda and
                x.dtype == torch.float32 and not x.requires_grad and
                os.environ.get("HCTR_SKINNY_FC", "1") != "0")

    def _layer(self, i, x):
        gw = self._gw[i] if self._gw else None
        gb = self._gb[i] if self._gb else None
        if i == 0 and self._skinny_first(x):
            return _SkinnyFirstFn.apply(x, self.weights[0], self.biases[0], self._w16[0],
                                        self._b16[0], gw, gb)
        if x.dtype != self.dtype:
            x = x.to(self.dtype)
        return _LinearFn.apply(x, self.weights[i], self.biases[i], self._w16[i], self._b16[i],
                               self.relu[i], self.wgrad_groups, gw, gb)

    def can_fuse_bce_head(self) -> bool:
        k = self.dims[-2]
        return (self.dims[-1] == 1 and not self.relu[-1] and k % 4 == 0 and k <= 2048 and
                self.dtype in _DT16)

    def forward_bce(self, x, label, grad_scale: float):
        assert self.can_fuse_bce_head()
        if not self._w16:
            self.refresh_shadow()
        n = len(self.weights)
        for i in range(n - 1):
            x = self._layer(i, x)
        if x.dtype != self.dtype:
            x = x.to(self.dtype)
        return _LogitHeadFn.apply(x, self.weights[-1], self.biases[-1], self._w16[-1], self._b16[-1],
                                  label, grad_scale, self._gw[-1] if self._gw else None,
                                  self._gb[-1] if self._gb else None)

    def forward(self, x):
        if not self._w16:
            self.refresh_shadow()
        for i in range(len(self.weights)):
            x = self._layer(i, x)
        return x
```

### hugectr_amd/hugectr.py

```python
from __future__ import annotations

import enum
import json
import os
import time
from dataclasses import dataclass, field
from typing import Dict, List, Optional, Sequence

import numpy as np
import torch
import torch.distributed as dist

from . import _lib
from .dense import FusedMLP, bce_with_logits
from .embedding import OptParams, SparseEmbeddingHash, backward_reorder, forward_reorder
from .embedding_collection import (DataParallelCollection, EmbeddingCollection,
                                   EmbeddingCollectionConfig, EmbeddingTableConfig)
from .metrics import EvalMetrics
from .layers import (MultiCrossLayer, interaction, interaction_gather, interaction_indexed,
                     regather_supported)
from .parallel import DistributedExchange, LocalizedExchange, reorder_row_map
from .parallel import all_reduce as _all_reduce
from . import data as _data


class Check_t(enum.Enum):
    Sum = 0
    Non = 1
    Unknown = 2


class DataReaderType_t(enum.Enum):
    Norm = 0
    Raw = 1
    Parquet = 2
    RawAsync = 3


class LrPolicy_t(enum.Enum):
    fixed = 0


class Optimizer_t(enum.IntEnum):
    Ftrl = 0
    Adam = 1
    RMSProp = 2
    AdaGrad = 3
    Nesterov = 4
    MomentumSGD = 5
    SGD = 6


class Update_t(enum.IntEnum):
    Local = 0
    Global = 1
    LazyGlobal = 2


class Embedding_t(enum.IntEnum):
    DistributedSlotSparseEmbeddingHash = 0
    LocalizedSlotSparseEmbeddingHash = 1


class Activation_t(enum.Enum):
    Relu = 0
    Non = 1
    Unspecified = 2


class Initializer_t(enum.Enum):
    Default = 0
    Uniform = 1
    XavierNorm = 2
    XavierUniform = 3
    Sinusoidal = 4
    Zero = 5


class Distribution_t(enum.Enum):
    Uniform = 0
    PowerLaw = 1


class PowerLaw_t(enum.Enum):
    Long = 0
    Medium = 1
    Short = 2
    Specific = 3


class MetricsType(enum.Enum):
    AUC = 0
    AverageLoss = 1
    HitRate = 2
    NDCG = 3
    SMAPE = 4


Layer_t = enum.Enum("Layer_t", [
    "BatchNorm", "LayerNorm", "BinaryCrossEntropyLoss", "Reshape", "Select", "Concat",
    "CrossEntropyLoss", "Dropout", "ELU", "InnerProduct", "MLP", "Interaction",
    "MultiCrossEntropyLoss", "ReLU", "ReLUHalf", "GRU", "MatrixMultiply", "MultiHeadAttention",
    "Scale", "FusedReshapeConcat", "FusedReshapeConcatGeneral", "Softmax", "PReLU_Dice",
    "ReduceMean", "Sub", "Gather", "Sigmoid", "Slice", "WeightMultiply", "FmOrder2", "Add",
    "ReduceSum", "MultiCross", "Cast", "ElementwiseMultiply", "SequenceMask", "Unknown"])


@dataclass
class Solver:
    model_name: str = ""
    seed: int = 0
    lr_policy: LrPolicy_t = LrPolicy_t.fixed
    lr: float = 0.001
    warmup_steps: int = 1
    decay_start: int = 0
    decay_steps: int = 1
    decay_power: float = 2.0
    end_lr: float = 0.0
    max_eval_batches: int = 100
    batchsize_eval: int = 2048
    batchsize: int = 2048
    vvgpu: List[List[int]] = field(default_factory=lambda: [[0]])
    repeat_dataset: bool = True
    use_mixed_precision: bool = False
    enable_tf32_compute: bool = False
    scaler: float = 1.0
    metrics_spec: Dict = field(default_factory=lambda: {MetricsType.AUC: 1.0})
    i64_input_key: bool = False
    use_algorithm_search: bool = True
    use_cuda_graph: bool = True
    gen_loss_summary: bool = True
    train_intra_iteration_overlap: bool = False
    train_inter_iteration_overlap: bool = False
    eval_intra_iteration_overlap: bool = False
    eval_inter_iteration_overlap: bool = False
    device_layout: str = "LOCAL_FIRST"
    use_embedding_collection: bool = False
    all_reduce_algo: str = "NCCL"
    grouped_all_reduce: bool = False
    num_iterations_statistics: int = 20
    perf_logging: bool = False
    drop_incomplete_batch: bool = True
    kafka_brockers: str = ""
    training_callbacks: list = field(default_factory=list)


def CreateSolver(**kw) -> Solver:
    s = Solver()
    for k, v in kw.items():
        if not hasattr(s, k):
            raise RuntimeError(f"CreateSolver: unknown argument '{k}'")
        setattr(s, k, v)
    if s.use_mixed_precision and s.scaler not in (128.0, 256.0, 512.0, 1024.0):
        raise RuntimeError("use_mixed_precision requires scaler in {128, 256, 512, 1024}")
    _launch_one_process_per_gpu(sum(len(v) for v in s.vvgpu))
    return s


def _launch_one_process_per_gpu(n_gpus: int):
    import sys
    if n_gpus <= 1 or "WORLD_SIZE" in os.environ or dist.is_initialized():
        return
    script = sys.argv[0] if sys.argv else ""
    main_file = getattr(sys.modules.get("__main__"), "__file__", None)
    direct = bool(main_file) and os.path.isfile(script) and \
        os.path.abspath(main_file) == os.path.abspath(script) and "pytest" not in sys.modules and \
        os.environ.get("HCTR_NO_RELAUNCH") != "1"
# ... 337 lines not shown
                               "launch one process per GPU (torch.distributed.run)")
        local = int(os.environ.get("LOCAL_RANK", "0"))
        if os.environ.get("HCTR_RANKS_ON_ONE_GPU") == "1":
            local = 0
        self.device = torch.device("cuda", local)
        torch.cuda.set_device(self.device)
        torch.manual_seed(solver.seed + 1)
        self.input: Optional[Input] = None
        self.embeddings: List[SparseEmbedding] = []
        self.ebc_configs: List[EmbeddingCollectionConfig] = []
        self.layers: List[DenseLayer] = []
        self._compiled = False
        self._loss = float("nan")
        self._lr = solver.lr
        self._iter = 0

    def add(self, item):
        if isinstance(item, Input):
            self.input = item
        elif isinstance(item, SparseEmbedding):
            self.embeddings.append(item)
        elif isinstance(item, EmbeddingCollectionConfig):
            self.ebc_configs.append(item)
        elif isinstance(item, DenseLayer):
            self.layers.append(item)
        else:
            raise RuntimeError(f"Model.add: unsupported item {type(item)}")

    def _emb_opt(self, se: SparseEmbedding) -> OptParams:
        o = se.optimizer if (se.optimizer is not None and se.optimizer.initialized) else self.opt
        return OptParams(optimizer=int(o.optimizer_type), update_type=int(o.update_type),
                         lr=self._lr, beta1=o.beta1, beta2=o.beta2, epsilon=o.epsilon,
                         initial_accu_value=o.initial_accu_value,
                         momentum_factor=o.momentum_factor,
                         atomic_update=bool(o.atomic_update) and
                         os.environ.get("HCTR_SGD_ATOMIC") == "1",
                         scaler=self.solver.scaler)

    def compile(self, loss_names=None, loss_weights=None):
        assert self.input is not None, "Model.add(Input(...)) first"
        self._loss_weights = dict(zip(self.input.label_names, self.input.label_weights))
        if loss_names is not None:
            ws = list(loss_weights) if loss_weights is not None else [1.0] * len(list(loss_names))
            if len(ws) != len(list(loss_names)):
                raise RuntimeError("compile: loss_names and loss_weights differ in length")
            for n, w in zip(loss_names, ws):
                if str(n) not in self.input.label_names:
                    raise RuntimeError(f"compile: '{n}' is not a label of this model "
                                       f"(labels: {self.input.label_names})")
                self._loss_weights[str(n)] = float(w)
        s = self.solver
        B, Be = s.batchsize, s.batchsize_eval
        self.bpg, self.bpg_eval = B // self.world, Be // self.world
        key_dtype = torch.int64 if s.i64_input_key else torch.uint32
        self.emb_dtype = torch.float16 if s.use_mixed_precision else torch.float32
        sp = {p.top_name: p for p in self.input.sparse_params}
        self._emb = {}
        self._shapes: Dict[str, tuple] = {self.input.dense_name: (self.input.dense_dim,)}
        for n, d in zip(self.input.label_names, self.input.label_dims):
            self._shapes[n] = (int(d),)
        for se in self.embeddings:
            p = sp[se.bottom_name]
            opt = self._emb_opt(se)
            ssa = se.slot_size_array or []
            if ssa:
                max_vocab = 0
            else:
                assert se.workspace_size_per_gpu_in_mb > 0, "workspace_size_per_gpu_in_mb or slot_size_array"
                max_vocab = _max_vocab_from_workspace(
                    se.workspace_size_per_gpu_in_mb,
                    se.optimizer if (se.optimizer is not None and se.optimizer.initialized)
                    else self.opt, se.embedding_vec_size)
            h = SparseEmbeddingHash(int(se.embedding_type), B, Be, max_vocab, se.embedding_vec_size,
                                    p.max_feature_num(), p.slot_num, se.combiner, opt,
                                    slot_size_array=ssa, key_dtype=key_dtype,
                                    out_dtype=self.emb_dtype, rank=self.rank, world=self.world,
                                    seed=s.seed, device=self.device)
            h.init_params()
            localized = se.embedding_type == Embedding_t.LocalizedSlotSparseEmbeddingHash
            ex = {}
            for mode, bb in (("train", B), ("eval", Be)):
                ex[mode] = (LocalizedExchange if localized else DistributedExchange)(
                    bb, p.slot_num, se.embedding_vec_size)
            self._emb[se.sparse_embedding_name] = (se, p, h, ex, localized)
            self._shapes[se.sparse_embedding_name] = (p.slot_num, se.embedding_vec_size)
        self._ebc = []
        for cfg in self.ebc_configs:
            subs = self._split_by_ev_size(cfg)
            if len(subs) == 1:
                subs[0][0].top_name = cfg.top_name
            for sub, ids in subs:
                rt = self._compile_ebc(sub, sp, B, Be, declare_shapes=len(subs) == 1)
                rt.update(parent=cfg, ids=ids, whole=len(subs) == 1)
                self._ebc.append(rt)
            if len(subs) > 1:
                def width(t, bottom, c):
                    h = sp[bottom].max_nnz() if str(c).lower().endswith("concat") else 1
                    return t.ev_size * max(h, 1)
                if cfg.top_name:
                    self._shapes[cfg.top_name] = (sum(width(t, b, c) for t, b, _, c in cfg.lookups),)
                else:
                    for t, b, top, c in cfg.lookups:
                        self._shapes[top] = (width(t, b, c),)
        self._mods = torch.nn.ModuleDict()
        self._loss_layer = None
        self._loss_layers = []
        for i, L in enumerate(self.layers):
            self._build_layer(i, L)
        self._mods.to(self.device)
        self._dense_params = [p for p in self._mods.parameters()]
        env = os.environ.get("HCTR_HIP_GRAPH", "auto")
        ebc_graph = bool(self.ebc_configs) and not self._emb and all(
            isinstance(rt["train"], EmbeddingCollection) for rt in self._ebc)
        self._graph_ok = (bool(s.use_cuda_graph) and env != "0" and self.world == 1 and
                          len(self._loss_layers) >= 1 and
                          ((not self.ebc_configs and len(self._loss_layers) == 1 and
                            (self.bpg <= 8192 or env == "1")) or
                           (ebc_graph and (self.bpg <= 32768 or env == "1"))))
        self._graph, self._graph_wait = None, 0
        self._dense_opt = self._make_dense_opt()
        self.reader = getattr(self, "reader_override", None) or _data.make_reader(
            self.reader_params, self.input, s, self.rank, self.world, self.device)
        self._gemm_selection = _use_gemm_selection(s)
        groups = [[p.top_name for p in rt["params"]] for rt in self._ebc]
        for j, rt in enumerate(self._ebc):
            rt["index"] = j
        for r in (getattr(self.reader, "train", None), getattr(self.reader, "evalr", None)):
            if r is not None and hasattr(r, "ebc_groups"):
                r.ebc_groups = groups
        self._plan_execution()
        self._metrics = EvalMetrics(s.metrics_spec, self.input.label_dim, self.bpg_eval,
                                    s.max_eval_batches, num_loss_layers=len(self._loss_layers),
                                    world=self.world, device=self.device)
        self._compiled = True

    def _plan_execution(self):
        s = self.solver
        consumers: Dict[str, list] = {}
        for i, L in enumerate(self.layers):
            for pos, b in enumerate(L.bottom_names):
                consumers.setdefault(b, []).append((i, pos))
        self._consumers = consumers
        fused_ok = os.environ.get("HCTR_MODEL_FUSED_DENSE", "1") != "0"
        mlps = [m for m in self._mods.values() if isinstance(m, FusedMLP)]
        in_mlps = sum(sum(q.numel() for q in m.parameters()) for m in mlps)
        total = sum(q.numel() for q in self._dense_params)
        self._flat_mlps = []
        if (fused_ok and mlps and in_mlps == total and s.use_mixed_precision and
                Optimizer_t(self.opt.optimizer_type) == Optimizer_t.SGD):
            for m in mlps:
                m.flatten()
            self._flat_mlps = mlps
            self._dense_opt = None
        self._head_layer = None
        if fused_ok and self._loss_layer is not None and s.use_mixed_precision:
            logit_name = self._loss_layer.bottom_names[0]
            for i, L in enumerate(self.layers):
                if (L.layer_type == Layer_t.MLP and L.top_names[0] == logit_name and
                        len(consumers.get(logit_name, [])) == 1 and
                        self._mods[f"l{i}"].can_fuse_bce_head()):
                    self._head_layer = i
        self._intra = bool(s.train_intra_iteration_overlap) and self.world > 1
        self._inter = bool(s.train_inter_iteration_overlap) and self.world > 1
        self._upd_overlap = bool(s.train_intra_iteration_overlap) and self.world == 1
        self._idx_mode = os.environ.get("HCTR_INDEX_AHEAD", "0")
        self._idx_overlap = (bool(s.train_inter_iteration_overlap) and self.world == 1 and
                             self._idx_mode != "0")
        want = os.environ.get("HCTR_EXCHANGE", "auto" if (self._intra and self._inter) else "rows")
        if want not in ("rows", "unique", "unique16", "auto"):
            raise RuntimeError("HCTR_EXCHANGE must be rows, unique, unique16 or auto")
        self._xstate = {}
        for name, (se, p, h, ex, localized) in self._emb.items():
            st = {"mode": "rows", "ux": None, "select": None, "indexed": False, "timing_ms": None,
                  "fused_gather": False, "rows_indexed": False}
            one_hot = p.is_fixed_length and p.max_nnz() == 1
            cons = consumers.get(name, [])
            to_interaction = (len(cons) == 1 and cons[0][1] == 1 and
                              self.layers[cons[0][0]].layer_type == Layer_t.Interaction)
            n_ins = p.slot_num + 1
            st["rows_indexed"] = (self.world > 1 and localized and to_interaction and
                                  s.use_mixed_precision and self._intra and
                                  se.embedding_vec_size in (32, 64, 128) and n_ins <= 32 and
                                  (se.embedding_vec_size + n_ins * (n_ins - 1) // 2 + 1) % 8 == 0 and
                                  os.environ.get("HCTR_ROWS_INDEXED", "1") != "0")
            if st["rows_indexed"]:
                st["row_map"] = reorder_row_map(self.bpg, p.slot_num, self.world).to(
                    self.device).contiguous()
            st["fused_gather"] = (self.world == 1 and one_hot and se.combiner == 0 and
                                  to_interaction and s.use_mixed_precision and
                                  se.embedding_vec_size in (16, 32, 64, 128) and p.slot_num <= 31 and
                                  os.environ.get("HCTR_FUSED_GATHER", "1") != "0")
            if (self.world > 1 and localized and one_hot and se.combiner == 0 and
                    want != "rows" and self._intra and
                    (se.embedding_vec_size * (2 if s.use_mixed_precision else 4)) % 16 == 0):
                try:
                    from .unique_exchange import UniqueExchange
                    st["ux"] = UniqueExchange(h, self.bpg, p.slot_num, se.embedding_vec_size)
                except Exception as e:
                    if self.rank == 0:
                        print(f"[HCTR][WARNING] unique-row exchange unavailable for {name}: {e!r}")
                if st["ux"] is not None:
                    st["indexed"] = to_interaction and s.use_mixed_precision
                    if want == "auto":
                        st["select"] = {"it": 0, "t0": 0.0, "t": {}}
                    else:
                        self._set_exchange(st, want)
            self._xstate[name] = st
        self._lookahead = None
        self._upd_stream = None
        self._idx_stream = None
        self._idx_ahead = {}
        self._upd_timing = []
        self._upd_overlap_on = True

    def _set_exchange(self, st, mode: str):
        st["mode"] = mode
        if st["ux"] is not None and mode != "rows":
            st["ux"].set_sum_dtype(self.emb_dtype if mode == "unique16" else torch.float32)

    _SEL_WARM, _SEL_TIMED, _SEL_SWITCH = 8, 3, 2

    def _select_exchange(self, st):
        sel = st["select"]
        W, T, S = self._SEL_WARM, self._SEL_TIMED, self._SEL_SWITCH
        it = sel["it"]
        sel["it"] += 1
        marks = {W: ("rows", None), W + T: ("unique", "rows"), W + T + S: ("unique", None),
                 W + 2 * T + S: (None, "unique")}
        if it not in marks:
            return
        nxt, done = marks[it]
        if done is not None or it in (W, W + T + S):
            if st["ux"] is not None:
                st["ux"].drain()
            torch.cuda.synchronize()
        if done is not None:
            sel["t"][done] = time.perf_counter() - sel["t0"]
        if it in (W, W + T + S):
            if dist.is_initialized():
                dist.barrier()
            sel["t0"] = time.perf_counter()
        if nxt is not None:
            self._set_exchange(st, nxt)
            return
        t = torch.tensor([sel["t"]["rows"], sel["t"]["unique"]], dtype=torch.float64)
        if dist.get_backend() != "gloo":
            t = t.to(self.device)
        dist.all_reduce(t, op=dist.ReduceOp.MAX)
        t = t.cpu()
        st["timing_ms"] = {"rows": float(t[0]) / T * 1e3, "unique": float(t[1]) / T * 1e3}
        self._set_exchange(st, "rows" if float(t[0]) <= float(t[1]) else "unique")
        st["select"] = None

    def exchange_report(self) -> dict:
        out = {}
        for name, (se, p, h, ex, localized) in self._emb.items():
            st = self._xstate[name]
            esz = 2 if self.solver.use_mixed_precision else 4
            D = se.embedding_vec_size
            r = {"payload": st["mode"] if self.world > 1 else "none (1 GPU)",
                 "gather_fused_into_interaction": st["fused_gather"],
                 "selection_ms_per_step": st["timing_ms"],
                 "intra_iteration_overlap": self._intra, "inter_iteration_overlap": self._inter}
            if self.world > 1 and localized and st["mode"] == "rows":
                e = ex["train"]
                r["bytes_out_forward"] = (sum(e.send) - e.send[self.rank]) * esz
                r["bytes_out_backward"] = (sum(e.recv) - e.recv[self.rank]) * esz
            elif self.world > 1 and st["ux"] is not None and st["ux"].u_send is not None:
                ux = st["ux"]
                us, ur = ux.u_send, ux.u_recv
                gsz = 2 if st["mode"] == "unique16" else 4
                r.update(distinct_rows_out=sum(us) - us[self.rank], positions=ux.P,
                         bytes_out_forward=(sum(us) - us[self.rank]) * D * esz +
                         (ux.P - ux.P // self.world) * 8,
                         bytes_out_backward=(sum(ur) - ur[self.rank]) * D * gsz)
            out[name] = r
        for i, rt in enumerate(getattr(self, "_ebc", [])):
            e = rt["train"]
            if getattr(e, "_unique", False):
                r = {"payload": "unique rows", "tables": [t.name for t in e.tables]}
                r.update(e.last_exchange or {})
                out[f"embedding_collection{i}"] = r
        return out

    def _split_by_ev_size(self, cfg: EmbeddingCollectionConfig):
        dp_names = set()
        if isinstance(cfg.shard_strategy, (list, tuple)):
            for kind, names in cfg.shard_strategy:
                if str(kind).lower() == "dp":
                    dp_names.update(str(n) for n in names)
        dp_names = {n for n in dp_names
                    if all(t.max_vocabulary_size >= 0 for t, _, _, _ in cfg.lookups if t.name == n)}
        sizes = sorted({t.ev_size for t, _, _, _ in cfg.lookups})
        comp = (getattr(cfg, "compression", None) or {}) if self.world > 1 else {}
        strategies = sorted({comp.get(t.name, "reduction") for t, _, _, _ in cfg.lookups
                             if t.name not in dp_names})
        def kind(t):
            return "hybrid" if getattr(t, "var_type", None) == "hybrid" else "plain"
        kinds = sorted({kind(t) for t, _, _, _ in cfg.lookups if t.name not in dp_names})
        if len(sizes) == 1 and not dp_names and len(strategies) <= 1 and len(kinds) <= 1:
            return [(cfg, list(range(len(cfg.lookups))))]
        tables = []
        for t, _, _, _ in cfg.lookups:
            if t not in tables:
                tables.append(t)
        own = cfg.ownership(tables, self.world)
# ... 453 lines not shown
            if localized:
                recv = ex[mode].forward(pooled)
                E = forward_reorder(recv, bpg, S, D, W) if W > 1 else pooled.view(bpg, S, D)
            else:
                E = h.forward_scale(train, ex[mode].forward(pooled).contiguous())
            if train:
                E = E.detach().requires_grad_(True)
                leaves[name] = E

                def finish(E=E):
                    g = E.grad
                    if os.environ.get("HCTR_DEBUG_LOSS_CURVE"):
                        self._last_emb_grad = g.detach().clone()
                    if localized and W > 1:
                        g = backward_reorder(g.contiguous(), bpg, S, D, W)
                    top = ex["train"].backward(g.contiguous())
                    h.backward(top.contiguous())
                    h.update_params()
                after.append(finish)
            tensors[name] = E
            return
        if st["mode"] != "rows":
            ux = st["ux"]
            ux.forward_begin(ro, keys)
            nk = nxt["sparse"][se.bottom_name] if (nxt is not None and self._inter) else None

            def resolve():
                if st["indexed"]:
                    rows, row_of = ux.forward_finish(indexed=True)
                    E = _IndexedEmb(rows, row_of, ux.backward_begin)
                else:
                    E = ux.forward_finish().detach().requires_grad_(True)
                    E.register_hook(lambda g: ux.backward_begin(g))
                if nk is not None:
                    ux.prefetch(*nk)
                return E
            tensors[name] = _Pending(resolve)
            after.append(ux.backward_finish)
            return
        pooled = h.forward(True, ro, keys)
        e = ex["train"]
        recv, work = e.forward_async(pooled)
        top_grad = torch.empty_like(pooled)
        sent = {}

        def on_grad(g):
            gsend = backward_reorder(g.contiguous(), bpg, S, D, W)
            sent["work"] = e.backward_async(gsend, top_grad.view(-1))
            sent["buf"] = gsend

        def on_rows_grad(gsend):
            sent["work"] = e.backward_async(gsend.view(-1), top_grad.view(-1))
            sent["buf"] = gsend

        def resolve():
            if work is not None:
                work.wait()
            if st["rows_indexed"]:
                return _IndexedEmb(recv.view(-1, D), st["row_map"], on_rows_grad, scatter=True)
            E = forward_reorder(recv, bpg, S, D, W).requires_grad_(True)
            E.register_hook(on_grad)
            return E

        def finish():
            if "work" not in sent:
                return
            if sent.get("work") is not None:
                sent["work"].wait()
            sent.clear()
            h.backward(top_grad)
            h.update_params()
        tensors[name] = _Pending(resolve)
        after.append(finish)

    def _ebc_tensors(self, tensors, rt, get_E):
        cfg = rt["parent"]
        span = getattr(rt["train"], "virt_span", None)

        parts = {}

        def piece(v0, reps, as_float=False):
            def resolve():
                E = get_E()
                if reps == 1:
                    if "u" not in parts:
                        parts["u"] = E.unbind(1)
                    x = parts["u"][v0]
                else:
                    x = E[:, v0:v0 + reps, :].reshape(E.shape[0], -1)
                return x.float() if as_float else x
            return _Pending(resolve)
        if rt["whole"]:
            if cfg.top_name:
                tensors[cfg.top_name] = _Pending(get_E)
            else:
                for l, (_, _, top, _) in enumerate(cfg.lookups):
                    v0, reps = span[l] if span else (l, 1)
                    tensors[top] = piece(v0, reps)
        else:
            for j, l in enumerate(rt["ids"]):
                v0, reps = span[j] if span else (j, 1)
                if cfg.top_name:
                    tensors[(id(cfg), l)] = piece(v0, reps, as_float=True)
                else:
                    tensors[cfg.lookups[l][2]] = piece(v0, reps)

    def _ebc_concat_tops(self, tensors):
        for cfg in self.ebc_configs:
            if cfg.top_name and dict.__contains__(tensors, (id(cfg), 0)):
                n = len(cfg.lookups)
                tensors[cfg.top_name] = _Pending(
                    lambda cfg=cfg, n=n: torch.cat([tensors[(id(cfg), l)] for l in range(n)], dim=1))

    def _multi_task_loss(self, tensors):
        total, probs = None, []
        for L, lg, lab in tensors["__logits__"]:
            w = self._loss_weights.get(L.bottom_names[1], 1.0)
            li = torch.nn.functional.binary_cross_entropy_with_logits(lg.float(), lab.float())
            total = li * w if total is None else total + li * w
            probs.append(torch.sigmoid(lg.float()))
        return total, probs

    def _run_batch(self, batch, train: bool, nxt=None):
        tensors = _Tensors({self.input.dense_name: batch["dense"]})
        off = 0
        for n, d in zip(self.input.label_names, self.input.label_dims):
            tensors[n] = batch["label"] if len(self.input.label_names) == 1 else \
                batch["label"][:, off:off + d]
            off += d
        leaves, after = {}, []
        for name in self._emb:
            self._emb_forward(name, batch, nxt, train, tensors, leaves, after)
        for i, rt in enumerate(self._ebc):
            self._ebc_tensors(tensors, rt, self._ebc_begin(rt, batch, train, after))
        self._ebc_concat_tops(tensors)
        label = batch["label"].float()
        gscale = self.solver.scaler / (max(self.bpg, 1) * self.world)
        head = (label, gscale) if (train and self._head_layer is not None and
                                   label.shape[1] == 1) else None
        multi = len(self._loss_layers) > 1
        if multi:
            head = None
        logit, loss = self._forward_dense(tensors, train, head)
        if multi:
            total, probs = self._multi_task_loss(tensors)
            if not train:
                return total, torch.cat(probs, dim=1)
            (total * (self.solver.scaler / self.world)).backward()
            loss = total
        elif not train:
            loss = torch.nn.functional.binary_cross_entropy_with_logits(logit, label)
            return loss, torch.sigmoid(logit)
        elif loss is not None:
            loss.backward()
        elif logit.is_cuda and label.shape == logit.shape:
            lg = tensors[self._loss_layer.bottom_names[0]]
            loss, dlogit = bce_with_logits(lg, label, gscale)
            lg.backward(dlogit)
        else:
            loss = torch.nn.functional.binary_cross_entropy_with_logits(logit, label)
            (loss * (self.solver.scaler / self.world)).backward()
        works = self._dense_reduce_begin()
        for fin in after:
            fin()
        self._dense_step(reduced=works)
        return loss.detach().reshape(()), None

    def _graph_dense(self, G, skip_step: bool):
        tensors = _Tensors({self.input.dense_name: G["dense"]})
        off = 0
        for n, d in zip(self.input.label_names, self.input.label_dims):
            tensors[n] = G["label"] if len(self.input.label_names) == 1 else \
                G["label"][:, off:off + d]
            off += d
        for name, (se, p, h, ex, localized) in self._emb.items():
            if self._xstate[name]["fused_gather"]:
                tensors[name] = _GatherEmb(h, True, lambda g, n=name: G["grads"].__setitem__(n, g))
            else:
                tensors[name] = G["leaf"][name]
        for i, rt in enumerate(self._ebc):
            self._ebc_tensors(tensors, rt, lambda i=i: G["ebc_leaf"][i])
        self._ebc_concat_tops(tensors)
        gscale = self.solver.scaler / max(self.bpg, 1)
        multi = len(self._loss_layers) > 1
        head = (G["label"], gscale) if (self._head_layer is not None and not multi and
                                        G["label"].shape[1] == 1) else None
        logit, loss = self._forward_dense(tensors, True, head)
        if multi:
            loss, _ = self._multi_task_loss(tensors)
            (loss * self.solver.scaler).backward()
        elif loss is not None:
            loss.backward()
        else:
            lg = tensors[self._loss_layer.bottom_names[0]]
            loss, dlogit = bce_with_logits(lg, G["label"], gscale)
            lg.backward(dlogit)
        for name, leaf in G["leaf"].items():
            G["grads"][name] = leaf.grad
        for i, leaf in enumerate(G["ebc_leaf"]):
            G["ebc_grads"][i] = leaf.grad
        self._dense_step(skip=skip_step)
        return loss.detach().reshape(())

    def _graph_capture(self, batch):
        B = self.bpg
        G = {"lr": self._lr, "leaf": {}, "pooled": {}, "grads": {}, "ebc_leaf": [], "ebc_grads": {},
             "dense": torch.empty_like(batch["dense"]),
             "label": torch.empty_like(batch["label"].float())}
        G["dense"].copy_(batch["dense"])
        G["label"].copy_(batch["label"].float())
        for rt in self._ebc:
            E = self._ebc_forward(rt, batch, True)
            G["ebc_leaf"].append(E.detach().clone().requires_grad_(True))
        for name, (se, p, h, ex, localized) in self._emb.items():
            ro, keys = batch["sparse"][se.bottom_name]
            if self._xstate[name]["fused_gather"]:
                h.index(True, ro, keys)
                continue
            S = h.slots_on_rank if localized else p.slot_num
            G["pooled"][name] = torch.empty((self.solver.batchsize, S, se.embedding_vec_size),
                                            dtype=self.emb_dtype, device=self.device)
            h.forward(True, ro, keys, out=G["pooled"][name])
            G["leaf"][name] = G["pooled"][name].view(B, p.slot_num, se.embedding_vec_size) \
                .requires_grad_(True)
        side = torch.cuda.Stream()
        side.wait_stream(torch.cuda.current_stream())
        with torch.cuda.stream(side):
            for _ in range(2):
                self._graph_dense(G, skip_step=True)
        torch.cuda.current_stream().wait_stream(side)
        for leaf in list(G["leaf"].values()) + G["ebc_leaf"]:
            leaf.grad = None
        for q in self._dense_params:
            q.grad = None
        G["graph"] = torch.cuda.CUDAGraph()
        with torch.cuda.graph(G["graph"]):
            G["loss"] = self._graph_dense(G, skip_step=False)
        return G

    def _graph_step(self, batch):
        G = self._graph
        fresh = G is None or G["lr"] != self._lr
        if fresh:
            G = self._graph = self._graph_capture(batch)
        else:
            for name, (se, p, h, ex, localized) in self._emb.items():
                ro, keys = batch["sparse"][se.bottom_name]
                if self._xstate[name]["fused_gather"]:
                    h.index(True, ro, keys)
                else:
                    h.forward(True, ro, keys, out=G["pooled"][name])
            for i, rt in enumerate(self._ebc):
                with torch.no_grad():
                    G["ebc_leaf"][i].copy_(self._ebc_forward(rt, batch, True))
            G["dense"].copy_(batch["dense"])
            G["label"].copy_(batch["label"])
        G["graph"].replay()
        for i, rt in enumerate(self._ebc):
            g = G["ebc_grads"].get(i)
            if g is not None:
                rt["train"].lr = self._lr
                rt["train"].backward_and_update(g.contiguous())
        for name, (se, p, h, ex, localized) in self._emb.items():
            g = G["grads"][name]
            if not self._xstate[name]["fused_gather"]:
                g = ex["train"].backward(g.contiguous())
            h.backward(g.contiguous())
            h.update_params()
        return G["loss"]

    def _dense_reduce_begin(self):
        if self.world == 1 or getattr(self, "_dense_frozen", False) or not self._intra or \
                dist.get_backend() == "gloo":
            return None
        ts = [m.flat_g for m in self._flat_mlps] if self._flat_mlps else \
            [q.grad for q in self._dense_params if q.grad is not None]
        return [dist.all_reduce(t, async_op=True) for t in ts]

    def _dense_step(self, skip: bool = False, reduced=None):
        frozen = getattr(self, "_dense_frozen", False) or skip
        if reduced is not None:
            for w in reduced:
                w.wait()
        if self._flat_mlps:
            if frozen:
                return
            for m in self._flat_mlps:
                if self.world > 1 and reduced is None:
                    _all_reduce(m.flat_g)
                m.sgd_step(self._lr, 1.0 / self.solver.scaler)
            return
        if self._dense_opt is None:
            return
        if frozen:
            self._dense_opt.zero_grad(set_to_none=True)
            return
        if self.world > 1 and reduced is None:
            for q in self._dense_params:
                if q.grad is not None:
                    _all_reduce(q.grad)
        if self.solver.scaler != 1.0:
            grads = [q.grad for q in self._dense_params if q.grad is not None]
            if grads:
                torch._foreach_div_(grads, self.solver.scaler)
        self._dense_opt.step()
        self._dense_opt.zero_grad(set_to_none=True)
        for m in self._mods.values():
            if isinstance(m, FusedMLP):
                m.refresh_shadow()

    def check_overflow(self, blocking: bool = True):
        if blocking:
            self._drain_prefetch()
        return self._check_overflow(blocking)

    def _check_overflow(self, blocking: bool = True):
        for (_, _, h, _, _) in self._emb.values():
            h.check_overflow() if blocking else h.poll_overflow()

    def train(self) -> bool:
        assert self._compiled
        for st in self._xstate.values():
            if st["select"] is not None:
                self._select_exchange(st)
        batch, self._lookahead = self._lookahead, None
        if batch is None:
            batch = self.reader.next_batch(train=True)
        if batch is None:
            return False
        nxt = None
        if (self._inter and any(st["mode"] != "rows" for st in self._xstate.values())) or \
                (self._idx_overlap and any(st["fused_gather"] for st in self._xstate.values())):
            nxt = self._lookahead = self.reader.next_batch(train=True)
        self.check_overflow(blocking=False)
        loss = None
        if self._graph_ok and not getattr(self, "_dense_frozen", False):
            if getattr(self, "_graph_lr", None) != self._lr:
                self._graph_lr, self._graph_wait, self._graph = self._lr, 3, None
            if self._graph_wait > 0:
                self._graph_wait -= 1
            else:
                try:
                    loss = self._graph_step(batch)
                except Exception as e:
                    if self._graph is not None:
                        raise
                    print(f"[HCTR][WARNING] HIP-graph capture failed ({e!r}); eager launches")
                    self._graph_ok = False
                    for q in self._dense_params:
                        q.grad = None
        if loss is None:
            loss, _ = self._run_batch(batch, True, nxt)
        self._loss_t = loss.detach()
        self._iter += 1
        return True

    def _drain_prefetch(self):
        for st in getattr(self, "_xstate", {}).values():
            if st["ux"] is not None:
                st["ux"].drain()
        for _, ev in getattr(self, "_idx_ahead", {}).values():
            torch.cuda.current_stream().wait_event(ev)

    @property
    def _eval_buf(self):
        return getattr(self, "_metrics", None)

    @_eval_buf.setter
    def _eval_buf(self, _):
        m = getattr(self, "_metrics", None)
        if m is not None:
            m.reset()

    def eval(self) -> bool:
        batch = self.reader.next_batch(train=False)
        if batch is None:
            return False
        self._drain_prefetch()
        if not self._eval_buf:
            self.check_overflow()
        with torch.no_grad():
            loss, prob = self._run_batch(batch, False)
        self._metrics.add_batch(prob, batch["label"], loss)
        return True

    def get_current_loss(self) -> float:
        return float(self._loss_t)

    def get_eval_metrics(self):
        return self._metrics.result()

    def set_learning_rate(self, lr: float):
        self._lr = lr
        for (_, _, h, _, _) in self._emb.values():
            h.set_learning_rate(lr)
        if self._dense_opt is not None:
            for g in self._dense_opt.param_groups:
                g["lr"] = lr

    def summary(self):
        if self.rank != 0:
            return
        print("=" * 67 + "Model Summary" + "=" * 67)
        print(f"{'Label':<40}{'Dense':<30}{'Sparse':<30}")
        print(f"{self.input.label_name:<40}{self.input.dense_name:<30}"
              f"{','.join(p.top_name for p in self.input.sparse_params):<30}")
        print(f"({self.bpg},{self.input.label_dim})".ljust(40) + f"({self.bpg},{self.input.dense_dim})")
        print("-" * 147)
        print(f"{'Layer Type':<40}{'Input Name':<30}{'Output Name':<30}{'Output Shape':<30}")
        for name, (se, p, h, _, _) in self._emb.items():
            print(f"{se.embedding_type.name:<40}{se.bottom_name:<30}{name:<30}"
                  f"({self.bpg},{p.slot_num},{se.embedding_vec_size})")
        for rt in self._ebc:
            cfg, e = rt["cfg"], rt["train"]
            print(f"{'EmbeddingCollection':<40}{','.join(b for _, b, _, _ in cfg.lookups)[:28]:<30}"
                  f"{(cfg.top_name or ','.join(t for _, _, t, _ in cfg.lookups))[:28]:<30}"
                  f"({self.bpg},{e.L},{e.ev})")
        for L in self.layers:
            tops = ",".join(L.top_names)
            shp = self._shapes.get(L.top_names[0], ()) if L.top_names else ()
            print(f"{L.layer_type.name:<40}{','.join(L.bottom_names):<30}{tops:<30}"
                  f"({self.bpg},{','.join(str(v) for v in shp)})")
        print("-" * 147)

    def fit(self, num_epochs=0, max_iter=2000, display=200, eval_interval=1000, snapshot=10000,
            snapshot_prefix="", data_source_params=None):
        assert self._compiled, "call compile() first"
        s = self.solver
        if self.rank == 0:
            print(f"=====================================================Model Fit====================="
                  f"================================")
            print(f"[HCTR][INFO] Use non-epoch mode with number of iterations: {max_iter}"
                  if num_epochs <= 0 else f"[HCTR][INFO] Use epoch mode with number of epochs: {num_epochs}")
            print(f"[HCTR][INFO] Training batchsize: {s.batchsize}, evaluation batchsize: {s.batchsize_eval}")
        t0 = t_fit = time.time()
        it = 0
        hit_target = False
        limit = max_iter if num_epochs <= 0 else 10 ** 12
        self._eval_buf = []
        callbacks = list(getattr(s, "training_callbacks", None) or [])
        for tc in callbacks:
# ... 420 lines not shown
```

### include/hugectr_amd.h

```cpp
#ifndef HUGECTR_AMD_H
#define HUGECTR_AMD_H
#include <stddef.h>
#include <stdint.h>

#ifdef __cplusplus
extern "C" {
#endif

typedef void* hctr_stream_t;

typedef enum {
  HCTR_OK = 0,
  HCTR_ERR_INVALID_ARG = -1,
  HCTR_ERR_HIP = -2,
  HCTR_ERR_OVERFLOW = -3,
  HCTR_ERR_UNSUPPORTED = -4,
  HCTR_ERR_IO = -5
} hctr_status;

typedef enum { HCTR_OPT_FTRL = 0, HCTR_OPT_ADAM = 1, HCTR_OPT_RMSPROP = 2, HCTR_OPT_ADAGRAD = 3,
               HCTR_OPT_NESTEROV = 4, HCTR_OPT_MOMENTUM_SGD = 5, HCTR_OPT_SGD = 6 } hctr_optimizer_t;
typedef enum { HCTR_UPDATE_LOCAL = 0, HCTR_UPDATE_GLOBAL = 1, HCTR_UPDATE_LAZY_GLOBAL = 2 } hctr_update_t;
typedef enum { HCTR_EMB_DISTRIBUTED_SLOT_HASH = 0, HCTR_EMB_LOCALIZED_SLOT_HASH = 1 } hctr_embedding_t;
typedef enum { HCTR_KEY_U32 = 0, HCTR_KEY_I64 = 1 } hctr_key_t;
// ... 190 lines not shown
int hctr_uniq_expand(size_t positions, int n_owners, const int64_t* q_off, const int64_t* r_off,
                     const uint32_t* meta, const void* rows, int vec_size, int dtype, void* out,
                     uint32_t* sorted_rows, uint32_t* sorted_buckets, uint32_t* row_of,
                     hctr_stream_t stream);
int hctr_updater_reduce_presorted(hctr_updater* u, size_t positions, size_t buckets,
                                  const int64_t* row_offset, const uint32_t* sorted_rows,
                                  const uint32_t* sorted_buckets, const void* grad, int grad_dtype,
                                  size_t n_rows, float* out_sum, hctr_stream_t stream);
size_t hctr_ebc_uniq_plan_workspace_bytes(size_t max_positions);
int hctr_ebc_uniq_plan(size_t positions, int world, size_t buckets_per_peer,
                       const int64_t* bucket_range, const uint64_t* rows, uint64_t max_row,
                       uint64_t* urow, int64_t* peer_off, uint32_t* ridx, void* workspace,
                       size_t workspace_bytes, hctr_stream_t stream);
int hctr_ebc_uniq_gather_rows(size_t n_rows, int ev_size, const uint64_t* urow, const float* table,
                              uint64_t row_bound, void* out, int out_dtype, hctr_stream_t stream);
int hctr_ebc_uniq_network_forward(size_t batch_per_gpu, int num_lookup, int ev_size, int max_shards,
                                  const int32_t* d_src_blocks, const int32_t* d_combiner,
                                  const int64_t* d_bucket_counts, int batch_major,
                                  const int64_t* recv_range, const uint32_t* ridx,
                                  const int64_t* r_off, const int32_t* d_block_source,
                                  const uint32_t* d_one_hot, const void* rows, void* out, int dtype,
                                  hctr_stream_t stream);
size_t hctr_ebc_uniq_backward_workspace_bytes(size_t max_positions, size_t batch_per_gpu,
                                              int num_lookup, int ev_size);
int hctr_ebc_uniq_network_backward(hctr_updater* u, size_t batch_per_gpu, int num_lookup,
                                   int ev_size, int num_blocks, const int32_t* d_block_lookup,
                                   const int32_t* d_block_source, const int32_t* d_combiner,
                                   const int64_t* d_bucket_counts, int batch_major, int any_average,
                                   const int64_t* recv_range, const uint32_t* ridx,
                                   const int64_t* r_off, size_t positions, size_t n_rows,
                                   const void* grad, int grad_dtype, float* out_sum,
                                   void* workspace, size_t workspace_bytes, hctr_stream_t stream);
int hctr_emb_index(hctr_embedding* emb, int is_train, const void* row_offset, const void* keys,
                   size_t nnz, hctr_stream_t stream);
int hctr_emb_index_ahead(hctr_embedding* emb, const void* row_offset, const void* keys, size_t nnz,
                         hctr_stream_t stream);
int hctr_emb_index_adopt(hctr_embedding* emb);
int hctr_emb_update_rows(hctr_embedding* emb, size_t n, const int64_t* row_offset,
                         const uint64_t* rows, const void* grad, int grad_dtype,
                         hctr_stream_t stream);

int hctr_interaction_fwd(size_t batch, int n_emb, int width, const void* mlp, const void* emb,
                         void* out, int dtype, hctr_stream_t stream);
int hctr_interaction_bwd(size_t batch, int n_emb, int width, const void* mlp, const void* emb,
                         const void* top_grad, void* mlp_grad, void* emb_grad, int dtype,
                         hctr_stream_t stream);

int hctr_interaction_fwd_indexed(size_t batch, int n_emb, int width, const void* mlp,
                                 const void* rows, const uint32_t* row_of, void* out, int dtype,
                                 hctr_stream_t stream);
int hctr_interaction_bwd_indexed(size_t batch, int n_emb, int width, const void* mlp,
                                 const void* rows, const uint32_t* row_of, const void* top_grad,
                                 void* mlp_grad, void* emb_grad, int dtype, hctr_stream_t stream);
int hctr_interaction_bwd_indexed_scatter(size_t batch, int n_emb, int width, const void* mlp,
                                         const void* rows, const uint32_t* row_of,
                                         const void* top_grad, void* mlp_grad, void* grad_rows,
                                         int dtype, hctr_stream_t stream);

int hctr_interaction_fwd_gather(size_t batch, int n_emb, int width, const void* mlp,
                                const float* table, const uint64_t* value_index, void* pooled,
                                void* out, int dtype, hctr_stream_t stream);
int hctr_interaction_bwd_gather(size_t batch, int n_emb, int width, const void* mlp,
                                const float* table, const uint64_t* value_index,
                                const void* top_grad, void* mlp_grad, void* emb_grad, int dtype,
                                hctr_stream_t stream);
int hctr_emb_forward_interaction(hctr_embedding* e, int is_train, const void* mlp, void* pooled,
                                 void* out, hctr_stream_t stream);
int hctr_emb_backward_interaction(hctr_embedding* e, const void* mlp, const void* top_grad,
                                  void* mlp_grad, void* emb_grad, hctr_stream_t stream);

int hctr_cross_v1_fwd(size_t batch, int width, int layers, const float* x0, const float* kernels,
                      const float* biases, float* outputs, float* hiddens, hctr_stream_t stream);
int hctr_cross_v1_bwd(size_t batch, int width, int layers, const float* x0, const float* kernels,
                      const float* outputs, const float* hiddens, const float* out_grad,
                      float* in_grad, float* kernel_grads, float* bias_grads, float* workspace,
                      hctr_stream_t stream);
size_t hctr_cross_v1_bwd_workspace_bytes(size_t batch, int width, int layers);

typedef struct hctr_det hctr_det;
int hctr_det_create(size_t num_classes, const size_t* dimension_per_class, const char* initializer,
                    size_t initial_capacity_per_class, int key_type, uint64_t seed,
                    hctr_det** out);
int hctr_det_destroy(hctr_det* h);
size_t hctr_det_num_classes(const hctr_det* h);
int hctr_det_lookup(hctr_det* h, const void* keys, float* elements, size_t num_keys,
                    const size_t* id_spaces, const size_t* id_space_offsets, size_t num_id_spaces,
                    hctr_stream_t stream);
int hctr_det_lookup_unsafe(hctr_det* h, const void* keys, float** elements, size_t num_keys,
                           const size_t* id_spaces, const size_t* id_space_offsets,
                           size_t num_id_spaces, hctr_stream_t stream);
int hctr_det_scatter_add(hctr_det* h, const void* keys, const float* elements, size_t num_keys,
                         const size_t* id_spaces, const size_t* id_space_offsets,
                         size_t num_id_spaces, hctr_stream_t stream);
int hctr_det_scatter_update(hctr_det* h, const void* keys, const float* elements, size_t num_keys,
                            const size_t* id_spaces, const size_t* id_space_offsets,
                            size_t num_id_spaces, hctr_stream_t stream);
int hctr_det_remove(hctr_det* h, const void* keys, size_t num_keys, const size_t* id_spaces,
                    const size_t* id_space_offsets, size_t num_id_spaces, hctr_stream_t stream);
int hctr_det_export(hctr_det* h, size_t class_index, void* keys, float* values, size_t num_keys,
                    size_t* exported, hctr_stream_t stream);
int hctr_det_lookup_index(hctr_det* h, size_t class_index, const void* keys, size_t num_keys,
                          int insert, uint64_t* row_index, hctr_stream_t stream);
int hctr_det_rows(hctr_det* h, size_t class_index, float** rows, size_t* capacity);
int hctr_det_row_store(hctr_det* h, float** rows, uint64_t* total_rows);
int hctr_det_state_store(hctr_det* h, int num_state, float** state0, float** state1,
                         hctr_stream_t stream);
int hctr_det_lookup_rows(hctr_det* h, const void* keys, size_t num_keys, const size_t* id_spaces,
                         const size_t* id_space_offsets, size_t num_id_spaces, int insert,
                         float** elements, uint64_t* row_index, uint64_t* class_row_base,
                         hctr_stream_t stream);
int hctr_det_clear(hctr_det* h, hctr_stream_t stream);
int hctr_det_size_per_class(hctr_det* h, size_t* sizes, hctr_stream_t stream);
int hctr_det_capacity_per_class(const hctr_det* h, size_t* capacities);
int hctr_det_repair_count(const hctr_det* h, uint64_t* out);

typedef struct {
  int optimizer;
  float lr, beta1, beta2, epsilon;
  float momentum_factor;
  float rmsprop_beta;
  float ftrl_lambda1, ftrl_lambda2, ftrl_beta;
  float scaler;
} hctr_det_opt_params;
int hctr_det_update(hctr_det* weights, hctr_det* states, const hctr_det_opt_params* p,
                    const void* unique_keys, size_t num_unique_keys, const size_t* id_spaces,
                    const size_t* id_space_offsets, size_t num_id_spaces,
                    const uint32_t* ev_start_indices, const float* wgrad, hctr_stream_t stream);

size_t hctr_relu_bwd_bias_workspace_bytes(size_t rows, int n);
int hctr_relu_bwd_bias(size_t rows, int n, const void* dy, const void* y, void* dz, float* db,
                       float* workspace, int dtype, hctr_stream_t stream);

int hctr_sum_groups(int groups, size_t n, const void* in, int dtype, float* out,
                    hctr_stream_t stream);

int hctr_sgd_shadow(size_t n, float lr, float grad_scale, float* w, const float* g, void* w16,
                    int dtype, hctr_stream_t stream);

size_t hctr_bce_loss_workspace_bytes(void);
int hctr_bce_loss(size_t batch, const void* logit, const float* label, float grad_scale,
                  void* dlogit, float* loss, float* workspace, int dtype, hctr_stream_t stream);

size_t hctr_logit_head_workspace_bytes(int k);
int hctr_logit_head(size_t batch, int k, const void* x, const void* w, const void* bias,
                    const float* label, float grad_scale, void* dx, float* dw, float* db,
                    float* loss, float* workspace, int dtype, hctr_stream_t stream);

int hctr_skinny_fc_fwd(size_t batch, int k, int n, const float* x, const void* w, const void* bias,
                       void* y, int dtype, hctr_stream_t stream);
size_t hctr_skinny_fc_bwd_workspace_bytes(int n);
int hctr_skinny_fc_bwd(size_t batch, int k, int n, const float* x, const void* dy, const void* y,
                       float* dw, float* db, float* workspace, int dtype, hctr_stream_t stream);

int hctr_gemm_nt16(size_t m, int n, int k, const void* a, int lda, const void* bt, int ldb, void* c,
                   int ldc, int epilogue, const void* bias, const void* x0, const void* xl,
                   void* h_out, int dtype, hctr_stream_t stream);
int hctr_convert_transpose16(size_t batch, int rows, int cols, const float* src, void* dst,
                             void* dst_t, int dtype, hctr_stream_t stream);
size_t hctr_cross_v2_bwd_step_workspace_bytes(size_t batch, int width);
int hctr_cross_v2_bwd_step(size_t batch, int width, const void* dy, const void* x0, const void* h,
                           void* acc, void* s0, float* db, float* workspace, int first, int dtype,
                           hctr_stream_t stream);

typedef struct hctr_cache hctr_cache;
int hctr_cache_create(size_t capacity_in_set, int vec_size, int key_type, hctr_cache** out);
int hctr_cache_destroy(hctr_cache* c);
size_t hctr_cache_capacity_in_set(const hctr_cache* c);
int hctr_cache_query(hctr_cache* c, const void* keys, size_t len, float* values,
                     uint64_t* missing_index, void* missing_keys, size_t* d_missing_len,
                     hctr_stream_t stream);
int hctr_cache_replace(hctr_cache* c, const void* keys, size_t len, const float* values,
                       hctr_stream_t stream);
int hctr_cache_update(hctr_cache* c, const void* keys, size_t len, const float* values,
                      hctr_stream_t stream);
int hctr_cache_dump(hctr_cache* c, void* keys, size_t* d_dump_counter, size_t start_set_index,
                    size_t end_set_index, hctr_stream_t stream);

typedef struct hctr_tiered hctr_tiered;
int hctr_tiered_create(size_t host_rows, int vec_size, size_t cache_capacity_in_set,
                       hctr_tiered** out);
int hctr_tiered_destroy(hctr_tiered* t);
float* hctr_tiered_host_rows(hctr_tiered* t);
hctr_cache* hctr_tiered_cache(hctr_tiered* t);
int hctr_tiered_lookup(hctr_tiered* t, const int64_t* keys, size_t len, float* out,
                       size_t* d_missing_len, hctr_stream_t stream);
int hctr_tiered_scatter(hctr_tiered* t, const int64_t* unique_keys, size_t len, const float* values,
                        int add, float alpha, hctr_stream_t stream);
int hctr_tiered_flush(hctr_tiered* t, hctr_stream_t stream);

typedef struct hctr_uvm hctr_uvm;
int hctr_uvm_create(size_t device_table_capacity, size_t host_table_capacity, size_t max_batch_size,
                    int vec_size, float default_value, int key_type, hctr_uvm** out);
int hctr_uvm_destroy(hctr_uvm* u);
hctr_tiered* hctr_uvm_tier(hctr_uvm* u);
int hctr_uvm_add(hctr_uvm* u, const void* h_keys, const float* h_vectors, size_t len);
int hctr_uvm_query(hctr_uvm* u, const void* d_keys, size_t len, float* d_vectors,
                   hctr_stream_t stream);
int hctr_uvm_clear(hctr_uvm* u, hctr_stream_t stream);
int hctr_uvm_lookup(hctr_uvm* u, const void* d_keys, size_t len, float* d_vectors,
                    uint64_t* d_row_index, size_t* d_missing_len, hctr_stream_t stream);
int hctr_uvm_scatter_rows(hctr_uvm* u, const uint64_t* d_unique_rows, size_t len,
                          const float* values, int add, float alpha, hctr_stream_t stream);
int hctr_uvm_check_overflow(hctr_uvm* u, hctr_stream_t stream);
int hctr_uvm_size(hctr_uvm* u, hctr_stream_t stream, size_t* out);

typedef struct hctr_lru hctr_lru;
int hctr_lru_create(size_t capacity, size_t bucket_size, int dim, int key_type,
                    const char* initializer, uint64_t seed, hctr_lru** out);
int hctr_lru_destroy(hctr_lru* h);
int hctr_lru_lookup_index(hctr_lru* h, const void* keys, size_t n, int insert, uint64_t* row_index,
                          void* evict_keys, float* evict_rows, size_t* n_evicted,
                          hctr_stream_t stream);
int hctr_lru_find(hctr_lru* h, const void* keys, size_t n, uint64_t* row_index,
                  hctr_stream_t stream);
int hctr_lru_rows(hctr_lru* h, float** rows, size_t* capacity);
int hctr_lru_state(hctr_lru* h, int i, float** state, hctr_stream_t stream);
int hctr_lru_export(hctr_lru* h, void* keys, uint64_t* slots, uint64_t* scores, float* rows,
                    size_t max_keys, size_t* exported, hctr_stream_t stream);
int hctr_lru_size(hctr_lru* h, size_t* out, hctr_stream_t stream);
int hctr_lru_rejected_count(hctr_lru* h, uint64_t* out, hctr_stream_t stream);
int hctr_lru_capacity(const hctr_lru* h, size_t* capacity, size_t* bucket_size);
#define HCTR_LRU_FILTERED 0xFFFFFFFFFFFFFFFEull
int hctr_lru_lookup_index_filtered(hctr_lru* h, const void* keys, size_t n, uint64_t admit_below,
                                   uint64_t* row_index, void* evict_keys, float* evict_rows,
                                   size_t* n_evicted, hctr_stream_t stream);
int hctr_lru_filtered_count(hctr_lru* h, uint64_t* out, hctr_stream_t stream);
int hctr_lru_compact(hctr_lru* h, size_t batch, size_t n, const long long* offsets,
                     const uint64_t* rows, const void* keys, const float* weights,
                     long long* out_offsets, uint64_t* out_rows, void* out_keys,
                     float* out_weights, size_t* n_kept, hctr_stream_t stream);
int hctr_lru_export_if(hctr_lru* h, uint64_t min_score, void* keys, uint64_t* slots,
                       uint64_t* scores, float* rows, size_t max_keys, size_t* exported,
                       size_t* matched, hctr_stream_t stream);
int hctr_lru_create_tiered(size_t capacity, size_t bucket_size, int dim, int key_type,
                           const char* initializer, uint64_t seed, size_t hbm_slots,
                           hctr_lru** out);
int hctr_lru_placement(const hctr_lru* h, size_t* hbm_slots, size_t* hbm_rows, size_t* host_rows);
int hctr_lru_host_part(const hctr_lru* h, int array, float** host);
int hctr_lru_gather_slots(hctr_lru* h, int array, const uint64_t* slots, size_t n, float* out,
                          hctr_stream_t stream);
int hctr_lru_scatter_slots(hctr_lru* h, int array, const uint64_t* slots, size_t n,
                           const float* values, int add, hctr_stream_t stream);
int hctr_lru_apply_update(hctr_lru* h, hctr_updater* u, size_t buckets, size_t nnz,
                          const int64_t* bucket_range, const uint64_t* slots, const void* grad,
                          int grad_dtype, int optimizer, float lr, float beta1, float beta2,
                          float epsilon, float momentum_factor, float scaler, uint64_t times,
                          hctr_stream_t stream);
int hctr_lru_create_growing(size_t init_capacity, size_t max_capacity, float max_load_factor,
                            size_t bucket_size, int dim, int key_type, const char* initializer,
                            uint64_t seed, size_t hbm_slots, hctr_lru** out);
int hctr_lru_growth(const hctr_lru* h, size_t* capacity_now, size_t* capacity_max,
                    uint64_t* doublings);


#define HCTR_DIST_SELECT_WS_BYTES(num_splits) ((size_t)8 * ((size_t)(num_splits) * 1024 + 1))
int hctr_dist_select(const void* keys, int key_type, size_t n, int num_splits, void* out_keys,
                     int32_t* order, int32_t* splits, void* workspace, size_t workspace_bytes,
                     hctr_stream_t stream);

#define HCTR_ROW_COPY_MAX_TASKS 32
typedef struct {
  const void* src;
  size_t src_rows;
  int dim;
  int index_type;
  const void* index;
  uint64_t index_div;
  size_t n;
  void* dst;
  size_t dst_rows;
  const int32_t* dst_pos;
} hctr_row_copy_task;
int hctr_indexed_row_copy(const hctr_row_copy_task* tasks, int num_tasks, int src_dtype,
                          int dst_dtype, hctr_stream_t stream);

typedef struct hctr_ebc_io hctr_ebc_io;
int hctr_ebc_io_create(size_t chunk_rows, int ev_size, int key_type, hctr_ebc_io** out);
int hctr_ebc_io_destroy(hctr_ebc_io* io);
int hctr_ebc_io_chunk(hctr_ebc_io* io, int which, void** keys, float** rows, float** state0,
                      float** state1);
int hctr_ebc_io_wait(hctr_ebc_io* io, int which);
int hctr_ebc_io_check(hctr_ebc_io* io, int which, size_t n, int num_shards, int shard_id,
                      uint64_t vocab, uint64_t* d_counts, hctr_stream_t stream);
int hctr_ebc_io_import_static(hctr_ebc_io* io, int which, size_t n, int num_shards, int shard_id,
                              uint64_t vocab, uint64_t row_start, float* table, float* state0,
                              float* state1, hctr_stream_t stream);
int hctr_ebc_io_select(hctr_ebc_io* io, int which, size_t n, int num_shards, int shard_id,
                       uint64_t vocab, int64_t* out_keys, float* out_rows, float* out_state0,
                       float* out_state1, size_t* selected, hctr_stream_t stream);
int hctr_ebc_io_scatter_rows(size_t n, int ev_size, const uint64_t* row_index, const float* src,
                             float* dst, uint64_t row_bound, hctr_stream_t stream);
int hctr_ebc_io_export_static(hctr_ebc_io* io, int which, size_t n, uint64_t first_key,
                              uint64_t key_step, const float* table_rows, const float* state0,
                              const float* state1, hctr_stream_t stream);

int hctr_ebc_group_segments(size_t n_seg, size_t seg_stride, const int64_t* seg_offsets,
                            const int64_t* seg_dst, const int64_t* keys, size_t nnz,
                            int64_t* out_keys, hctr_stream_t stream);
int hctr_ebc_hybrid_row_ptrs(size_t n_seg, size_t seg_stride, const int64_t* seg_offsets,
                             const int64_t* seg_dst, const int32_t* seg_table, int n_tables,
                             const uint64_t* table_desc, int ev_size, const uint64_t* rows,
                             size_t nnz, const float** out_ptrs, uint32_t* out_perm,
                             hctr_stream_t stream);
int hctr_ebc_hybrid_key_grads(size_t buckets, int ev_size, const int64_t* bucket_range,
                              const uint32_t* perm, size_t nnz, const void* grad, int grad_dtype,
                              size_t samples, size_t lookups, float* key_grads,
// ... 21 lines not shown
```

Measured before the change: 30.45 million samples/s.

## Fuse dense gradient reductions and SGD update into one segmented finish kernel

The per-layer gradient finishing kernels (group sums, bias column sums, logit-head and skinny-FC partial reductions) are deferred and merged into a single segmented kernel driven by a device-side segment table. On one GPU that kernel also applies SGD and writes the fp16/bf16 shadow weights directly, so the separate gradient write and sgd_shadow pass go away. The goal is fewer kernel launches and less memory traffic over the dense gradients in each step, paid for with a table rebuild whenever the segment layout changes and a more complex code path. The loss backward also reuses a cached ones tensor instead of allocating one every step.

```diff
diff --git a/hugectr_amd/_lib.py b/hugectr_amd/_lib.py
--- a/hugectr_amd/_lib.py
+++ b/hugectr_amd/_lib.py
@@ -220,6 +220,14 @@
     "hctr_skinny_fc_fwd": (c_int, [c_size_t, c_int, c_int, _P, _P, _P, _P, c_int, _P]),
     "hctr_skinny_fc_bwd_workspace_bytes": (c_size_t, [c_int]),
     "hctr_skinny_fc_bwd": (c_int, [c_size_t, c_int, c_int, _P, _P, _P, _P, _P, _P, c_int, _P]),
+    "hctr_relu_bwd_bias_partials": (c_int, [c_size_t, c_int, _P, _P, _P, _P, c_int, _P]),
+    "hctr_logit_head_blocks": (c_int, [c_size_t, c_int]),
+    "hctr_logit_head_partials": (c_int, [c_size_t, c_int, _P, _P, _P, _P, c_float, _P, _P, c_int,
+                                         _P]),
+    "hctr_skinny_fc_bwd_blocks": (c_int, [c_size_t, c_int, c_int, _P, _P]),
+    "hctr_skinny_fc_bwd_partials": (c_int, [c_size_t, c_int, c_int, _P, _P, _P, _P, c_int, _P]),
+    "hctr_dense_seg_blocks": (c_int, [c_int, c_size_t]),
+    "hctr_dense_grad_finish": (c_int, [_P, c_int, c_size_t, c_int, c_float, c_float, _P, _P]),
     "hctr_sum_groups": (c_int, [c_int, c_size_t, _P, c_int, _P, _P]),
     "hctr_sgd_shadow": (c_int, [c_size_t, c_float, c_float, _P, _P, _P, c_int, _P]),
     "hctr_bce_loss_workspace_bytes": (c_size_t, []),
diff --git a/hugectr_amd/csrc/dense_ops.hip b/hugectr_amd/csrc/dense_ops.hip
--- a/hugectr_amd/csrc/dense_ops.hip
+++ b/hugectr_amd/csrc/dense_ops.hip
@@ -311,6 +311,12 @@
   o[1] = f32x4{acc[4], acc[5], acc[6], acc[7]};
 }
 
+template <typename V>
+__device__ __forceinline__ V sgd_apply(V w, V g, float lr, float grad_scale) {
+  w -= lr * grad_scale * g;
+  return w;
+}
+
 template <bool BF>
 __global__ void __launch_bounds__(kBlock)
     sgd_shadow_kernel(size_t n4, float lr, float grad_scale, float* __restrict__ w,
@@ -320,7 +326,7 @@
        i += (size_t)gridDim.x * kBlock) {
     f32x4 wv = reinterpret_cast<f32x4*>(w)[i];
     const f32x4 gv = reinterpret_cast<const f32x4*>(g)[i];
-    wv -= lr * grad_scale * gv;
+    wv = sgd_apply(wv, gv, lr, grad_scale);
     reinterpret_cast<f32x4*>(w)[i] = wv;
     const unsigned lo = (unsigned)H::from_f32(wv[0]) | ((unsigned)H::from_f32(wv[1]) << 16);
     const unsigned hi = (unsigned)H::from_f32(wv[2]) | ((unsigned)H::from_f32(wv[3]) << 16);
@@ -757,6 +763,179 @@
     const int n = i / stride, k = i % stride;
     if (k == kSkinnyK) db[n] = tot;
     else if (k < K) dw[(size_t)n * K + k] = tot;
+  }
+}
+
+template <bool SGD>
+__device__ __forceinline__ void finish_store4(const hctr_dense_seg& sg, size_t at, f32x4 gv,
+                                              float lr, float grad_scale) {
+  if (!SGD) {
+    *reinterpret_cast<f32x4*>(reinterpret_cast<float*>(sg.g) + at) = gv;
+    return;
+  }
+  f32x4* wp = reinterpret_cast<f32x4*>(reinterpret_cast<float*>(sg.w) + at);
+  const f32x4 wv = sgd_apply(*wp, gv, lr, grad_scale);
+  *wp = wv;
+  unsigned lo, hi;
+  if (sg.bf16) {
+    lo = (unsigned)H16<true>::from_f32(wv[0]) | ((unsigned)H16<true>::from_f32(wv[1]) << 16);
+    hi = (unsigned)H16<true>::from_f32(wv[2]) | ((unsigned)H16<true>::from_f32(wv[3]) << 16);
+  } else {
+    lo = (unsigned)H16<false>::from_f32(wv[0]) | ((unsigned)H16<false>::from_f32(wv[1]) << 16);
+    hi = (unsigned)H16<false>::from_f32(wv[2]) | ((unsigned)H16<false>::from_f32(wv[3]) << 16);
+  }
+  *reinterpret_cast<uint2*>(reinterpret_cast<unsigned short*>(sg.w16) + at) = make_uint2(lo, hi);
+}
+
+template <bool SGD>
+__device__ __forceinline__ void finish_store1(const hctr_dense_seg& sg, size_t at, float gv,
+                                              float lr, float grad_scale) {
+  if (!SGD) {
+    reinterpret_cast<float*>(sg.g)[at] = gv;
+    return;
+  }
+  float* wp = reinterpret_cast<float*>(sg.w) + at;
+  const float wv = sgd_apply(*wp, gv, lr, grad_scale);
+  *wp = wv;
+  reinterpret_cast<unsigned short*>(sg.w16)[at] =
+      sg.bf16 ? H16<true>::from_f32(wv) : H16<false>::from_f32(wv);
+}
+
+template <bool BF>
+__device__ __forceinline__ void finish_sum_groups(int groups, size_t n8, size_t i,
+                                                  const unsigned short* __restrict__ in,
+                                                  f32x4& lo, f32x4& hi) {
+  using H = H16<BF>;
+  float acc[8] = {0.f, 0.f, 0.f, 0.f, 0.f, 0.f, 0.f, 0.f};
+#pragma unroll 16
+  for (int g = 0; g < groups; g++) {
+    const u32x4 v = *reinterpret_cast<const u32x4*>(in + ((size_t)g * n8 + i) * 8);
+#pragma unroll
+    for (int e = 0; e < 4; e++) {
+      acc[2 * e] += H::to_f32((unsigned short)(v[e] & 0xFFFFu));
+      acc[2 * e + 1] += H::to_f32((unsigned short)(v[e] >> 16));
+    }
+  }
+  lo = f32x4{acc[0], acc[1], acc[2], acc[3]};
+  hi = f32x4{acc[4], acc[5], acc[6], acc[7]};
+}
+
+__device__ __forceinline__ float finish_block_chunks(float (*part)[64], int blocks, size_t stride,
+                                                     size_t col, bool live,
+                                                     const float* __restrict__ partial) {
+  const int c = threadIdx.x & 63;
+  const int chunk = (blocks + 15) / 16;
+  for (int grp = threadIdx.x >> 6; grp < 16; grp += kBlock / 64) {
+    const int b0 = grp * chunk, b1 = min(blocks, b0 + chunk);
+    float t = 0.f;
+    if (live) {
+      int b = b0;
+      for (; b + 8 <= b1; b += 8) {
+        float v[8];
+#pragma unroll
+        for (int u = 0; u < 8; u++) v[u] = partial[(size_t)(b + u) * stride + col];
+#pragma unroll
+        for (int u = 0; u < 8; u++) t += v[u];
+      }
+      for (; b < b1; b++) t += partial[(size_t)b * stride + col];
+    }
+    part[grp][c] = t;
+  }
+  __syncthreads();
+  float tot = 0.f;
+  if (threadIdx.x < 64 && live) {
+#pragma unroll
+    for (int g = 0; g < 16; g++) tot += part[g][c];
+  }
+  return tot;
+}
+
+template <bool SGD>
+__global__ void __launch_bounds__(kBlock)
+    dense_grad_finish_kernel(const hctr_dense_seg* __restrict__ segs, int nseg, float lr,
+                             float grad_scale, float* __restrict__ loss) {
+  __shared__ f32x4 red[kBlock];
+  int si = -1;
+  for (int base = 0; base < nseg; base += 64) {
+    const int t = base + (int)(threadIdx.x & 63);
+    const bool in = t < nseg && segs[t].block0 <= (long long)blockIdx.x;
+    si += (int)__popcll(__ballot(in));
+  }
+  const hctr_dense_seg sg = segs[si];
+  const int blk = (int)((long long)blockIdx.x - sg.block0);
+  const size_t dst = (size_t)sg.dst, dst2 = (size_t)sg.dst2;
+  switch ((int)sg.kind) {
+    case HCTR_DENSE_SEG_SUM_GROUPS: {
+      const size_t n8 = (size_t)sg.n / 8;
+      const size_t i = (size_t)blk * kBlock + threadIdx.x;
+      if (i >= n8) return;
+      const unsigned short* in = reinterpret_cast<const unsigned short*>(sg.src);
+      f32x4 lo, hi;
+      if (sg.src_bf16) finish_sum_groups<true>((int)sg.count, n8, i, in, lo, hi);
+      else finish_sum_groups<false>((int)sg.count, n8, i, in, lo, hi);
+      finish_store4<SGD>(sg, dst + i * 8, lo, lr, grad_scale);
+      finish_store4<SGD>(sg, dst + i * 8 + 4, hi, lr, grad_scale);
+      return;
+    }
+    case HCTR_DENSE_SEG_COLSUM: {
+      const float* partial = reinterpret_cast<const float*>(sg.src);
+      const size_t tiles = (size_t)sg.count;
+      const int n = (int)sg.n;
+      const int c4 = blk * 8 + (threadIdx.x & 7), tg = threadIdx.x >> 3;
+      const bool live = c4 * 4 < n;
+      f32x4 s = {0.f, 0.f, 0.f, 0.f};
+      if (live) {
+#pragma unroll 8
+        for (size_t t = tg; t < tiles; t += 32)
+          s += *reinterpret_cast<const f32x4*>(partial + t * n + c4 * 4);
+      }
+      red[threadIdx.x] = s;
+      __syncthreads();
+      if (tg == 0 && live) {
+        f32x4 sum = {0.f, 0.f, 0.f, 0.f};
+#pragma unroll
+        for (int k = 0; k < 32; k++) sum += red[k * 8 + threadIdx.x];
+        finish_store4<SGD>(sg, dst + (size_t)c4 * 4, sum, lr, grad_scale);
+      }
+      return;
+    }
+    case HCTR_DENSE_SEG_LOGIT_HEAD: {
+      const int K = (int)sg.n;
+      const int k = blk * 64 + (int)(threadIdx.x & 63);
+      const bool live = k < K + 2;
+      const float tot = finish_block_chunks(reinterpret_cast<float(*)[64]>(red), (int)sg.count,
+                                            (size_t)(K + 2), (size_t)k, live,
+                                            reinterpret_cast<const float*>(sg.src));
+      if (threadIdx.x < 64 && live) {
+        if (k < K) finish_store1<SGD>(sg, dst + k, tot, lr, grad_scale);
+        else if (k == K) finish_store1<SGD>(sg, dst2, tot, lr, grad_scale);
+        else if (loss) *loss = tot / (float)(size_t)sg.k;
+      }
+      return;
+    }
+    case HCTR_DENSE_SEG_SKINNY: {
+      const int stride = kSkinnyK + 1;
+      const int K = (int)sg.k, total = (int)sg.n * stride;
+      const int i = blk * 64 + (int)(threadIdx.x & 63);
+      const bool live = i < total;
+      const float tot = finish_block_chunks(reinterpret_cast<float(*)[64]>(red), (int)sg.count,
+                                            (size_t)total, (size_t)i, live,
+                                            reinterpret_cast<const float*>(sg.src));
+      if (threadIdx.x < 64 && live) {
+        const int n = i / stride, kk = i % stride;
+        if (kk == kSkinnyK) finish_store1<SGD>(sg, dst2 + n, tot, lr, grad_scale);
+        else if (kk < K) finish_store1<SGD>(sg, dst + (size_t)n * K + kk, tot, lr, grad_scale);
+      }
+      return;
+    }
+    default: {
+      if (!SGD) return;
+      const size_t i = (size_t)blk * kBlock + threadIdx.x;
+      if (i >= (size_t)sg.n / 4) return;
+      const f32x4 gv = *reinterpret_cast<const f32x4*>(reinterpret_cast<const float*>(sg.g) + dst + i * 4);
+      finish_store4<SGD>(sg, dst + i * 4, gv, lr, grad_scale);
+      return;
+    }
   }
 }
 
@@ -841,12 +1020,12 @@
   return ceil_div<size_t>(rows, (size_t)kRbRows) * (size_t)n * sizeof(float);
 }
 
-int hctr_relu_bwd_bias(size_t rows, int n, const void* dy, const void* y, void* dz, float* db,
-                       float* workspace, int dtype, hctr_stream_t stream) {
+static int relu_bwd_bias_impl(size_t rows, int n, const void* dy, const void* y, void* dz, float* db,
+                              float* workspace, int dtype, bool finish, hctr_stream_t stream) {
   HCTR_REQUIRE(n > 0 && n % 8 == 0, "n must be a multiple of 8");
   HCTR_REQUIRE(dtype == HCTR_EMB_BF16 || dtype == HCTR_EMB_F16, "16-bit dtypes only");
   if (rows == 0) return HCTR_OK;
-  HCTR_REQUIRE(dy && y && dz && db && workspace, "null pointer");
+  HCTR_REQUIRE(dy && y && dz && (db || !finish) && workspace, "null pointer");
   hipStream_t s = as_stream(stream);
   const size_t tiles = ceil_div<size_t>(rows, (size_t)kRbRows);
   const int cw = n / 8 < kBlock ? n / 8 : kBlock;
@@ -860,10 +1039,21 @@
                        rows, n, cw, rg, (const unsigned short*)dy, (const unsigned short*)y,
                        (unsigned short*)dz, workspace);
   HCTR_LAUNCH_CHECK();
+  if (!finish) return HCTR_OK;
   hipLaunchKernelGGL(colsum_partials_kernel, dim3(ceil_div<int>(n, 32)), dim3(kBlock), 0, s,
                      tiles, n, workspace, db);
   HCTR_LAUNCH_CHECK();
   return HCTR_OK;
+}
+
+int hctr_relu_bwd_bias(size_t rows, int n, const void* dy, const void* y, void* dz, float* db,
+                       float* workspace, int dtype, hctr_stream_t stream) {
+  return relu_bwd_bias_impl(rows, n, dy, y, dz, db, workspace, dtype, true, stream);
+}
+
+int hctr_relu_bwd_bias_partials(size_t rows, int n, const void* dy, const void* y, void* dz,
+                                float* workspace, int dtype, hctr_stream_t stream) {
+  return relu_bwd_bias_impl(rows, n, dy, y, dz, nullptr, workspace, dtype, false, stream);
 }
 
 size_t hctr_cross_v2_bwd_step_workspace_bytes(size_t batch, int width) {
@@ -977,21 +1167,33 @@
 
 size_t hctr_logit_head_workspace_bytes(int k) { return (size_t)kHeadBlocks * (k + 2) * sizeof(float); }
 
-int hctr_logit_head(size_t batch, int k, const void* x, const void* w, const void* bias,
-                    const float* label, float grad_scale, void* dx, float* dw, float* db,
-                    float* loss, float* workspace, int dtype, hctr_stream_t stream) {
+static int logit_head_rows(int k) {
+  const int nseg = (k + 255) / 256;
+  return nseg <= 1 ? 8 : (nseg <= 2 ? 4 : (nseg <= 4 ? 2 : 1));
+}
+
+int hctr_logit_head_blocks(size_t batch, int k) {
+  HCTR_REQUIRE(batch > 0 && k >= 4 && k % 4 == 0 && k <= 256 * kHeadMaxSeg,
+               "logit head: K must be a multiple of 4 and <= 2048");
+  return (int)std::min<size_t>((size_t)kHeadBlocks,
+                               ceil_div<size_t>(batch, (size_t)(kBlock / 64) * logit_head_rows(k)));
+}
+
+static int logit_head_impl(size_t batch, int k, const void* x, const void* w, const void* bias,
+                           const float* label, float grad_scale, void* dx, float* dw, float* db,
+                           float* loss, float* workspace, int dtype, bool finish,
+                           hctr_stream_t stream) {
   HCTR_REQUIRE(batch > 0 && k >= 4 && k % 4 == 0 && k <= 256 * kHeadMaxSeg,
                "logit head: K must be a multiple of 4 and <= 2048");
   HCTR_REQUIRE(dtype == HCTR_EMB_F16 || dtype == HCTR_EMB_BF16, "16-bit activations");
-  HCTR_REQUIRE(x && w && bias && label && dw && db && loss && workspace, "null pointer");
+  HCTR_REQUIRE(x && w && bias && label && ((dw && db && loss) || !finish) && workspace,
+               "null pointer");
   HCTR_REQUIRE(reinterpret_cast<uintptr_t>(x) % 8 == 0 && reinterpret_cast<uintptr_t>(w) % 8 == 0 &&
                    (dx == nullptr || reinterpret_cast<uintptr_t>(dx) % 8 == 0),
                "8-byte aligned buffers");
   hipStream_t s = as_stream(stream);
   const int nseg = (k + 255) / 256;
-  const int rows = nseg <= 1 ? 8 : (nseg <= 2 ? 4 : (nseg <= 4 ? 2 : 1));
-  const int blocks = (int)std::min<size_t>(
-      (size_t)kHeadBlocks, ceil_div<size_t>(batch, (size_t)(kBlock / 64) * rows));
+  const int blocks = hctr_logit_head_blocks(batch, k);
   const size_t lds = (size_t)(kBlock / 64) * (k + 2) * sizeof(float);
 #define HCTR_HEAD(T_, NSEG_, ROWS_)                                                               \
   hipLaunchKernelGGL((logit_head_kernel<T_, NSEG_, ROWS_>), dim3(blocks), dim3(kBlock), lds, s,   \
@@ -1010,10 +1212,25 @@
 #undef HCTR_HEAD_T
 #undef HCTR_HEAD
   HCTR_LAUNCH_CHECK();
+  if (!finish) return HCTR_OK;
   hipLaunchKernelGGL(logit_head_finish_kernel, dim3(ceil_div<int>(k + 2, 64)), dim3(1024), 0, s,
                      blocks, k, batch, workspace, dw, db, loss);
   HCTR_LAUNCH_CHECK();
   return HCTR_OK;
+}
+
+int hctr_logit_head(size_t batch, int k, const void* x, const void* w, const void* bias,
+                    const float* label, float grad_scale, void* dx, float* dw, float* db,
+                    float* loss, float* workspace, int dtype, hctr_stream_t stream) {
+  return logit_head_impl(batch, k, x, w, bias, label, grad_scale, dx, dw, db, loss, workspace,
+                         dtype, true, stream);
+}
+
+int hctr_logit_head_partials(size_t batch, int k, const void* x, const void* w, const void* bias,
+                             const float* label, float grad_scale, void* dx, float* workspace,
+                             int dtype, hctr_stream_t stream) {
+  return logit_head_impl(batch, k, x, w, bias, label, grad_scale, dx, nullptr, nullptr, nullptr,
+                         workspace, dtype, false, stream);
 }
 
 static int skinny_check(size_t batch, int k, int n, int dtype) {
@@ -1048,21 +1265,38 @@
   return (size_t)kSkinnyBlocks * n * (kSkinnyK + 1) * sizeof(float);
 }
 
-int hctr_skinny_fc_bwd(size_t batch, int k, int n, const float* x, const void* dy, const void* y,
-                       float* dw, float* db, float* workspace, int dtype, hctr_stream_t stream) {
+static int skinny_bwd_blocks(size_t batch, int k, int n, const void* dy, const void* y, bool* mfma) {
+  const char* mode = getenv("HCTR_SKINNY_BWD");
+  const bool want_mfma = mode ? strcmp(mode, "valu") != 0 : kSkinnyBwdMfmaDefault;
+  *mfma = want_mfma && k < kSkinnyK && n % 8 == 0 && reinterpret_cast<uintptr_t>(dy) % 16 == 0 &&
+          reinterpret_cast<uintptr_t>(y) % 16 == 0;
+  if (*mfma) {
+    const int rsets = (kSkinnyBwdBlock / 64) / ceil_div<int>(n, 128);
+    return (int)std::min<size_t>((size_t)kSkinnyBlocks, ceil_div<size_t>(batch, (size_t)rsets * 16));
+  }
+  return (int)std::min<size_t>((size_t)kSkinnyBlocks,
+                               ceil_div<size_t>(batch, kSkinnyBwdBlock / kSkinnyLanes));
+}
+
+int hctr_skinny_fc_bwd_blocks(size_t batch, int k, int n, const void* dy, const void* y) {
+  HCTR_REQUIRE(batch > 0 && k >= 1 && k <= kSkinnyK, "skinny fc: 1 <= K <= 16");
+  HCTR_REQUIRE(n >= 4 && n % 4 == 0 && n <= 512, "skinny fc: N a multiple of 4, <= 512");
+  bool mfma;
+  return skinny_bwd_blocks(batch, k, n, dy, y, &mfma);
+}
+
+static int skinny_fc_bwd_impl(size_t batch, int k, int n, const float* x, const void* dy,
+                              const void* y, float* dw, float* db, float* workspace, int dtype,
+                              bool finish, hctr_stream_t stream) {
   HCTR_TRY(skinny_check(batch, k, n, dtype));
-  HCTR_REQUIRE(x && dy && y && dw && db && workspace, "null pointer");
+  HCTR_REQUIRE(x && dy && y && ((dw && db) || !finish) && workspace, "null pointer");
   HCTR_REQUIRE(reinterpret_cast<uintptr_t>(dy) % 8 == 0 && reinterpret_cast<uintptr_t>(y) % 8 == 0,
                "8-byte aligned activations");
   hipStream_t s = as_stream(stream);
   const size_t lds = (size_t)n * (kSkinnyK + 1) * sizeof(float);
-  const char* mode = getenv("HCTR_SKINNY_BWD");
-  const bool want_mfma = mode ? strcmp(mode, "valu") != 0 : kSkinnyBwdMfmaDefault;
-  if (want_mfma && k < kSkinnyK && n % 8 == 0 && reinterpret_cast<uintptr_t>(dy) % 16 == 0 &&
-      reinterpret_cast<uintptr_t>(y) % 16 == 0) {
-    const int rsets = (kSkinnyBwdBlock / 64) / ceil_div<int>(n, 128);
-    const int blocks = (int)std::min<size_t>((size_t)kSkinnyBlocks,
-                                             ceil_div<size_t>(batch, (size_t)rsets * 16));
+  bool mfma;
+  const int blocks = skinny_bwd_blocks(batch, k, n, dy, y, &mfma);
+  if (mfma) {
     if (dtype == HCTR_EMB_BF16)
       hipLaunchKernelGGL(skinny_fc_bwd_mfma_kernel<__hip_bfloat16>, dim3(blocks),
                          dim3(kSkinnyBwdBlock), lds, s, batch, k, n, x, (const __hip_bfloat16*)dy,
@@ -1071,13 +1305,12 @@
       hipLaunchKernelGGL(skinny_fc_bwd_mfma_kernel<__half>, dim3(blocks), dim3(kSkinnyBwdBlock), lds,
                          s, batch, k, n, x, (const __half*)dy, (const __half*)y, workspace);
     HCTR_LAUNCH_CHECK();
+    if (!finish) return HCTR_OK;
     hipLaunchKernelGGL(skinny_fc_finish_kernel, dim3(ceil_div<int>(n * (kSkinnyK + 1), 64)),
                        dim3(1024), 0, s, blocks, k, n, workspace, dw, db);
     HCTR_LAUNCH_CHECK();
     return HCTR_OK;
   }
-  const int blocks = (int)std::min<size_t>(
-      (size_t)kSkinnyBlocks, ceil_div<size_t>(batch, kSkinnyBwdBlock / kSkinnyLanes));
   if (dtype == HCTR_EMB_BF16)
     hipLaunchKernelGGL(skinny_fc_bwd_kernel<__hip_bfloat16>, dim3(blocks), dim3(kSkinnyBwdBlock), lds, s,
                        batch, k, n, x, (const __hip_bfloat16*)dy, (const __hip_bfloat16*)y,
@@ -1086,10 +1319,49 @@
     hipLaunchKernelGGL(skinny_fc_bwd_kernel<__half>, dim3(blocks), dim3(kSkinnyBwdBlock), lds, s, batch, k, n,
                        x, (const __half*)dy, (const __half*)y, workspace);
   HCTR_LAUNCH_CHECK();
+  if (!finish) return HCTR_OK;
   hipLaunchKernelGGL(skinny_fc_finish_kernel, dim3(ceil_div<int>(n * (kSkinnyK + 1), 64)),
                      dim3(1024), 0, s, blocks, k, n, workspace, dw, db);
   HCTR_LAUNCH_CHECK();
   return HCTR_OK;
 }
 
-}
+int hctr_skinny_fc_bwd(size_t batch, int k, int n, const float* x, const void* dy, const void* y,
+                       float* dw, float* db, float* workspace, int dtype, hctr_stream_t stream) {
+  return skinny_fc_bwd_impl(batch, k, n, x, dy, y, dw, db, workspace, dtype, true, stream);
+}
+
+int hctr_skinny_fc_bwd_partials(size_t batch, int k, int n, const float* x, const void* dy,
+                                const void* y, float* workspace, int dtype, hctr_stream_t stream) {
+  return skinny_fc_bwd_impl(batch, k, n, x, dy, y, nullptr, nullptr, workspace, dtype, false,
+                            stream);
+}
+
+int hctr_dense_seg_blocks(int kind, size_t n) {
+  switch (kind) {
+    case HCTR_DENSE_SEG_SUM_GROUPS: return (int)ceil_div<size_t>(n / 8, (size_t)kBlock);
+    case HCTR_DENSE_SEG_COLSUM: return (int)ceil_div<size_t>(n, 32);
+    case HCTR_DENSE_SEG_LOGIT_HEAD: return (int)ceil_div<size_t>(n + 2, 64);
+    case HCTR_DENSE_SEG_SKINNY: return (int)ceil_div<size_t>(n * (kSkinnyK + 1), 64);
+    case HCTR_DENSE_SEG_DIRECT: return (int)ceil_div<size_t>(n / 4, (size_t)kBlock);
+    default: HCTR_REQUIRE(false, "dense finish: unknown segment kind");
+  }
+}
+
+int hctr_dense_grad_finish(const hctr_dense_seg* segs, int nseg, size_t nblocks, int sgd, float lr,
+                           float grad_scale, float* loss, hctr_stream_t stream) {
+  HCTR_REQUIRE(nseg >= 0 && nblocks <= 0x7FFFFFFFu, "dense finish: segment / block count");
+  if (nseg == 0 || nblocks == 0) return HCTR_OK;
+  HCTR_REQUIRE(segs, "null pointer");
+  hipStream_t s = as_stream(stream);
+  if (sgd)
+    hipLaunchKernelGGL(dense_grad_finish_kernel<true>, dim3((unsigned)nblocks), dim3(kBlock), 0, s,
+                       segs, nseg, lr, grad_scale, loss);
+  else
+    hipLaunchKernelGGL(dense_grad_finish_kernel<false>, dim3((unsigned)nblocks), dim3(kBlock), 0, s,
+                       segs, nseg, lr, grad_scale, loss);
+  HCTR_LAUNCH_CHECK();
+  return HCTR_OK;
+}
+
+}
diff --git a/hugectr_amd/dense.py b/hugectr_amd/dense.py
--- a/hugectr_amd/dense.py
+++ b/hugectr_amd/dense.py
@@ -12,21 +12,40 @@
 _DT = {torch.float32: 0, torch.float16: 1, torch.bfloat16: 2}
 
 
-def split_k_wgrad(dy: torch.Tensor, x: torch.Tensor, groups: int = 16,
-                  out: torch.Tensor = None) -> torch.Tensor:
-    B, o = dy.shape
-    i = x.shape[1]
+def _count(rc: int) -> int:
+    if rc < 0:
+        check(rc)
+    return rc
+
+
+def _split_k_groups(B: int, o: int, i: int, groups: int) -> int:
     g = groups
     while g > 1 and B % g != 0:
         g //= 2
-    if g <= 1 or min(o, i) < 8:
+    return g if g > 1 and min(o, i) >= 8 else 0
+
+
+def split_k_wgrad(dy: torch.Tensor, x: torch.Tensor, groups: int = 16,
+                  out: torch.Tensor = None, part: torch.Tensor = None,
+                  finish: bool = True):
+    B, o = dy.shape
+    i = x.shape[1]
+    g = _split_k_groups(B, o, i, groups)
+    if g == 0:
         r = dy.t() @ x
         if out is not None:
             out.copy_(r)
             return out
         return r
-    p = torch.bmm(dy.view(g, B // g, o).transpose(1, 2), x.view(g, B // g, i))
-    if p.is_cuda and p.dtype in _DT16 and (o * i) % 8 == 0:
+    a, b = dy.view(g, B // g, o).transpose(1, 2), x.view(g, B // g, i)
+    hip = dy.is_cuda and dy.dtype in _DT16 and (o * i) % 8 == 0
+    if hip and part is not None and part.dtype == dy.dtype:
+        p = torch.bmm(a, b, out=part[:g * o * i].view(g, o, i))
+        if not finish:
+            return g
+    else:
+        p = torch.bmm(a, b)
+    if hip:
         if out is None:
             out = torch.empty((o, i), dtype=torch.float32, device=p.device)
         check(lib.hctr_sum_groups(g, o * i, ptr(p), _DT16[p.dtype], ptr(out), stream_ptr()))
@@ -50,12 +69,33 @@
     return loss, dlogit
 
 
+_SEG_SUM, _SEG_COLSUM, _SEG_HEAD, _SEG_SKINNY, _SEG_DIRECT = range(5)
+
+
+class _LayerWS:
+
+    def __init__(self, mlp, idx: int, wpart: torch.Tensor):
+        self.mlp, self.idx, self.wpart = mlp, idx, wpart
+        self._ws = None
+        self.w_seg = self.b_seg = None
+
+    @property
+    def defer(self) -> bool:
+        return self.mlp._finisher is not None
+
+    def ws(self, nbytes: int) -> torch.Tensor:
+        if self._ws is None or self._ws.numel() * 4 < nbytes:
+            self._ws = torch.empty(nbytes // 4, dtype=torch.float32, device=self.wpart.device)
+        return self._ws
+
+
 class _LinearFn(torch.autograd.Function):
 
     @staticmethod
-    def forward(ctx, x, w_master, b_master, w16, b16, relu: bool, groups: int, gw=None, gb=None):
+    def forward(ctx, x, w_master, b_master, w16, b16, relu: bool, groups: int, gw=None, gb=None,
+                lw=None):
         x = x.contiguous()
-        ctx.gw, ctx.gb = gw, gb
+        ctx.gw, ctx.gb, ctx.lw = gw, gb, lw
         if relu:
             y = torch._addmm_activation(b16, x, w16.t(), use_gelu=False)
         else:
@@ -69,14 +109,25 @@
         x, w16, y = ctx.saved_tensors
         dy = dy.contiguous()
         n = dy.shape[1]
+        lw = ctx.lw
+        defer = lw is not None and lw.defer
+        if lw is not None:
+            lw.w_seg = lw.b_seg = None
         if ctx.relu and n % 8 == 0 and dy.dtype in _DT16 and dy.is_cuda:
             dz = torch.empty_like(dy)
-            db = ctx.gb if ctx.gb is not None else torch.empty(n, dtype=torch.float32,
-                                                             device=dy.device)
-            ws = torch.empty(lib.hctr_relu_bwd_bias_workspace_bytes(dy.shape[0], n) // 4,
-                             dtype=torch.float32, device=dy.device)
-            check(lib.hctr_relu_bwd_bias(dy.shape[0], n, ptr(dy), ptr(y), ptr(dz), ptr(db), ptr(ws),
-                                         _DT16[dy.dtype], stream_ptr()))
+            nbytes = lib.hctr_relu_bwd_bias_workspace_bytes(dy.shape[0], n)
+            ws = lw.ws(nbytes) if lw is not None else \
+                torch.empty(nbytes // 4, dtype=torch.float32, device=dy.device)
+            if defer:
+                check(lib.hctr_relu_bwd_bias_partials(dy.shape[0], n, ptr(dy), ptr(y), ptr(dz),
+                                                      ptr(ws), _DT16[dy.dtype], stream_ptr()))
+                lw.b_seg = (_SEG_COLSUM, ws, nbytes // (4 * n), 0)
+                db = None
+            else:
+                db = ctx.gb if ctx.gb is not None else torch.empty(n, dtype=torch.float32,
+                                                                 device=dy.device)
+                check(lib.hctr_relu_bwd_bias(dy.shape[0], n, ptr(dy), ptr(y), ptr(dz), ptr(db),
+                                             ptr(ws), _DT16[dy.dtype], stream_ptr()))
             dy = dz
         else:
             if ctx.relu:
@@ -85,16 +136,19 @@
             if ctx.gb is not None:
                 ctx.gb.copy_(db)
         dx = dy @ w16 if ctx.needs_input_grad[0] else None
-        dw = split_k_wgrad(dy, x, ctx.groups, out=ctx.gw)
+        dw = split_k_wgrad(dy, x, ctx.groups, out=ctx.gw, part=lw.wpart if lw is not None else None,
+                           finish=not defer)
+        if defer and isinstance(dw, int):
+            lw.w_seg = (_SEG_SUM, lw.wpart, dw, 0)
         if ctx.gw is not None:
-            return dx, None, None, None, None, None, None, None, None
-        return dx, dw.float(), db, None, None, None, None, None, None
+            return dx, None, None, None, None, None, None, None, None, None
+        return dx, dw.float(), db, None, None, None, None, None, None, None
 
 
 class _SkinnyFirstFn(torch.autograd.Function):
 
     @staticmethod
-    def forward(ctx, x, w_master, b_master, w16, b16, gw=None, gb=None):
+    def forward(ctx, x, w_master, b_master, w16, b16, gw=None, gb=None, lw=None):
         x = x.contiguous()
         B, K = x.shape
         N = w16.shape[0]
@@ -104,7 +158,7 @@
                                          _DT16[w16.dtype], stream_ptr()))
         else:
             y = torch._addmm_activation(b16, x.to(w16.dtype), w16.t(), use_gelu=False)
-        ctx.gw, ctx.gb = gw, gb
+        ctx.gw, ctx.gb, ctx.lw = gw, gb, lw
         ctx.save_for_backward(x, y)
         return y
 
@@ -115,35 +169,59 @@
         B, K = x.shape
         N = y.shape[1]
         dev = x.device
+        lw = ctx.lw
+        nbytes = lib.hctr_skinny_fc_bwd_workspace_bytes(N)
+        ws = lw.ws(nbytes) if lw is not None else \
+            torch.empty(nbytes // 4, dtype=torch.float32, device=dev)
+        if lw is not None and lw.defer:
+            check(lib.hctr_skinny_fc_bwd_partials(B, K, N, ptr(x), ptr(dy), ptr(y), ptr(ws),
+                                                  _DT16[y.dtype], stream_ptr()))
+            blocks = _count(lib.hctr_skinny_fc_bwd_blocks(B, K, N, ptr(dy), ptr(y)))
+            lw.w_seg, lw.b_seg = (_SEG_SKINNY, ws, blocks, K), None
+            return None, None, None, None, None, None, None, None
+        if lw is not None:
+            lw.w_seg = lw.b_seg = None
         dw = ctx.gw if ctx.gw is not None else torch.empty((N, K), dtype=torch.float32, device=dev)
         db = ctx.gb if ctx.gb is not None else torch.empty(N, dtype=torch.float32, device=dev)
-        ws = torch.empty(lib.hctr_skinny_fc_bwd_workspace_bytes(N) // 4, dtype=torch.float32,
-                         device=dev)
         check(lib.hctr_skinny_fc_bwd(B, K, N, ptr(x), ptr(dy), ptr(y), ptr(dw), ptr(db), ptr(ws),
                                      _DT16[y.dtype], stream_ptr()))
         if ctx.gw is not None:
-            return None, None, None, None, None, None, None
-        return None, dw, db, None, None, None, None
+            return None, None, None, None, None, None, None, None
+        return None, dw, db, None, None, None, None, None
 
 
 class _LogitHeadFn(torch.autograd.Function):
 
     @staticmethod
-    def forward(ctx, x, w_master, b_master, w16, b16, label, grad_scale: float, gw=None, gb=None):
+    def forward(ctx, x, w_master, b_master, w16, b16, label, grad_scale: float, gw=None, gb=None,
+                lw=None):
         x = x.contiguous()
         B, K = x.shape
         dev = x.device
         dx = torch.empty_like(x) if ctx.needs_input_grad[0] else None
+        loss = torch.empty(1, dtype=torch.float32, device=dev)
+        nbytes = lib.hctr_logit_head_workspace_bytes(K)
+        ws = lw.ws(nbytes) if lw is not None else \
+            torch.empty(nbytes // 4, dtype=torch.float32, device=dev)
+        label = label.contiguous()
+        ctx.flat = gw is not None
+        ctx.dx = dx
+        if lw is not None and lw.defer:
+            check(lib.hctr_logit_head_partials(B, K, ptr(x), ptr(w16), ptr(b16), ptr(label),
+                                               float(grad_scale), ptr(dx), ptr(ws), _DT16[x.dtype],
+                                               stream_ptr()))
+            lw.w_seg = (_SEG_HEAD, ws, _count(lib.hctr_logit_head_blocks(B, K)), B)
+            lw.b_seg = None
+            lw.mlp._loss_out = loss
+            ctx.dw = ctx.db = None
+            return loss
+        if lw is not None:
+            lw.w_seg = lw.b_seg = None
         dw = gw if gw is not None else torch.empty((1, K), dtype=torch.float32, device=dev)
         db = gb if gb is not None else torch.empty(1, dtype=torch.float32, device=dev)
-        loss = torch.empty(1, dtype=torch.float32, device=dev)
-        ws = torch.empty(lib.hctr_logit_head_workspace_bytes(K) // 4, dtype=torch.float32, device=dev)
-        label = label.contiguous()
         check(lib.hctr_logit_head(B, K, ptr(x), ptr(w16), ptr(b16), ptr(label),
                                   float(grad_scale), ptr(dx), ptr(dw), ptr(db), ptr(loss), ptr(ws),
                                   _DT16[x.dtype], stream_ptr()))
-        ctx.flat = gw is not None
-        ctx.dx = dx
         ctx.dw, ctx.db = (None, None) if ctx.flat else (dw, db)
         return loss
 
@@ -151,7 +229,7 @@
     def backward(ctx, _grad_loss):
         dx, dw, db = ctx.dx, ctx.dw, ctx.db
         ctx.dx = ctx.dw = ctx.db = None
-        return dx, dw, db, None, None, None, None, None, None
+        return dx, dw, db, None, None, None, None, None, None, None
 
 
 class FusedMLP(torch.nn.Module):
@@ -174,6 +252,9 @@
         self.flat_w = self.flat_g = self.flat_w16 = None
         self._gw: List[torch.Tensor] = []
         self._gb: List[torch.Tensor] = []
+        self._lw: List[_LayerWS] = []
+        self._finisher = None
+        self._loss_out = None
 
     def flatten(self):
         dev = self.weights[0].device
@@ -198,6 +279,14 @@
         gviews = [self.flat_g[o:o + n].view_as(p) for p, o, n in zip(params, offs, sizes)]
         self._gw, self._gb = gviews[:nl], gviews[nl:]
         self.flat_w16.copy_(self.flat_w)
+        self._offs = (offs[:nl], offs[nl:])
+        need = [self.wgrad_groups * w.numel() if min(w.shape) >= 8 else 0 for w in self.weights]
+        starts, at = [], 0
+        for n in need:
+            starts.append(at)
+            at += (n + 255) // 256 * 256
+        part = torch.empty(max(at, 1), dtype=self.dtype, device=dev)
+        self._lw = [_LayerWS(self, i, part[starts[i]:starts[i] + need[i]]) for i in range(nl)]
         return self
 
     def sgd_step(self, lr: float, grad_scale: float = 1.0):
@@ -226,13 +315,14 @@
     def _layer(self, i, x):
         gw = self._gw[i] if self._gw else None
         gb = self._gb[i] if self._gb else None
+        lw = self._lw[i] if self._lw else None
         if i == 0 and self._skinny_first(x):
             return _SkinnyFirstFn.apply(x, self.weights[0], self.biases[0], self._w16[0],
-                                        self._b16[0], gw, gb)
+                                        self._b16[0], gw, gb, lw)
         if x.dtype != self.dtype:
             x = x.to(self.dtype)
         return _LinearFn.apply(x, self.weights[i], self.biases[i], self._w16[i], self._b16[i],
-                               self.relu[i], self.wgrad_groups, gw, gb)
+                               self.relu[i], self.wgrad_groups, gw, gb, lw)
 
     def can_fuse_bce_head(self) -> bool:
         k = self.dims[-2]
@@ -250,7 +340,8 @@
             x = x.to(self.dtype)
         return _LogitHeadFn.apply(x, self.weights[-1], self.biases[-1], self._w16[-1], self._b16[-1],
                                   label, grad_scale, self._gw[-1] if self._gw else None,
-                                  self._gb[-1] if self._gb else None)
+                                  self._gb[-1] if self._gb else None,
+                                  self._lw[-1] if self._lw else None)
 
     def forward(self, x):
         if not self._w16:
@@ -258,3 +349,71 @@
         for i in range(len(self.weights)):
             x = self._layer(i, x)
         return x
+
+
+class DenseGradFinish:
+
+    _FIELDS = 16
+
+    def __init__(self, mlps: Sequence["FusedMLP"]):
+        self.mlps = list(mlps)
+        for m in self.mlps:
+            assert m.flat_w is not None, "DenseGradFinish: flatten() the module first"
+            m._finisher = self
+        self._sig = None
+        self._table = None
+        self._nseg = self._nblocks = 0
+
+    def release(self):
+        for m in self.mlps:
+            m._finisher = None
+
+    def _segments(self):
+        segs = []
+        for m in self.mlps:
+            base = (m.flat_g.data_ptr(), m.flat_w.data_ptr(), m.flat_w16.data_ptr(),
+                    int(m.dtype == torch.bfloat16))
+            offw, offb = m._offs
+            for i, lw in enumerate(m._lw):
+                nw, nb = m.weights[i].numel(), m.biases[i].numel()
+                ws, bs = lw.w_seg, lw.b_seg
+                if ws is None:
+                    segs.append((_SEG_DIRECT, 0, 0, (nw + 3) // 4 * 4, 0, offw[i], 0, 0) + base)
+                elif ws[0] == _SEG_SUM:
+                    segs.append((_SEG_SUM, ws[1].data_ptr(), ws[2], nw, 0, offw[i], 0,
+                                 int(ws[1].dtype == torch.bfloat16)) + base)
+                elif ws[0] == _SEG_HEAD:
+                    segs.append((_SEG_HEAD, ws[1].data_ptr(), ws[2], nw, ws[3], offw[i], offb[i],
+                                 0) + base)
+                else:
+                    segs.append((_SEG_SKINNY, ws[1].data_ptr(), ws[2], nb, ws[3], offw[i], offb[i],
+                                 0) + base)
+                if ws is not None and ws[0] in (_SEG_HEAD, _SEG_SKINNY):
+                    continue
+                if bs is None:
+                    segs.append((_SEG_DIRECT, 0, 0, (nb + 3) // 4 * 4, 0, offb[i], 0, 0) + base)
+                else:
+                    segs.append((_SEG_COLSUM, bs[1].data_ptr(), bs[2], nb, 0, offb[i], 0, 0) + base)
+        return tuple(segs)
+
+    def _build(self, segs):
+        import numpy as np
+        t = np.zeros((len(segs), self._FIELDS), dtype=np.int64)
+        block0 = 0
+        for r, (kind, src, count, n, k, dst, dst2, src_bf, g, w, w16, bf) in enumerate(segs):
+            t[r, :13] = (kind, src, count, n, k, block0, g, w, w16, dst, dst2, bf, src_bf)
+            block0 += _count(lib.hctr_dense_seg_blocks(kind, n))
+        self._table = torch.from_numpy(t).to(self.mlps[0].flat_w.device)
+        self._nseg, self._nblocks = len(segs), block0
+
+    def finish(self, sgd: bool, lr: float = 0.0, grad_scale: float = 1.0):
+        segs = self._segments()
+        if segs != self._sig:
+            self._build(segs)
+            self._sig = segs
+        loss = None
+        for m in self.mlps:
+            if m._loss_out is not None:
+                loss, m._loss_out = m._loss_out, None
+        check(lib.hctr_dense_grad_finish(ptr(self._table), self._nseg, self._nblocks, int(sgd),
+                                         float(lr), float(grad_scale), ptr(loss), stream_ptr()))
diff --git a/hugectr_amd/hugectr.py b/hugectr_amd/hugectr.py
--- a/hugectr_amd/hugectr.py
+++ b/hugectr_amd/hugectr.py
@@ -12,7 +12,7 @@
 import torch.distributed as dist
 
 from . import _lib
-from .dense import FusedMLP, bce_with_logits
+from .dense import DenseGradFinish, FusedMLP, bce_with_logits
 from .embedding import OptParams, SparseEmbeddingHash, backward_reorder, forward_reorder
 from .embedding_collection import (DataParallelCollection, EmbeddingCollection,
                                    EmbeddingCollectionConfig, EmbeddingTableConfig)
@@ -656,6 +656,7 @@
                 m.flatten()
             self._flat_mlps = mlps
             self._dense_opt = None
+            self._dense_finish = DenseGradFinish(mlps)
         self._head_layer = None
         if fused_ok and self._loss_layer is not None and s.use_mixed_precision:
             logit_name = self._loss_layer.bottom_names[0]
@@ -1415,7 +1416,7 @@
             loss = torch.nn.functional.binary_cross_entropy_with_logits(logit, label)
             return loss, torch.sigmoid(logit)
         elif loss is not None:
-            loss.backward()
+            loss.backward(self._unit_grad(loss))
         elif logit.is_cuda and label.shape == logit.shape:
             lg = tensors[self._loss_layer.bottom_names[0]]
             loss, dlogit = bce_with_logits(lg, label, gscale)
@@ -1453,7 +1454,7 @@
             loss, _ = self._multi_task_loss(tensors)
             (loss * self.solver.scaler).backward()
         elif loss is not None:
-            loss.backward()
+            loss.backward(self._unit_grad(loss))
         else:
             lg = tensors[self._loss_layer.bottom_names[0]]
             loss, dlogit = bce_with_logits(lg, G["label"], gscale)
@@ -1536,9 +1537,17 @@
         if self.world == 1 or getattr(self, "_dense_frozen", False) or not self._intra or \
                 dist.get_backend() == "gloo":
             return None
+        if self._flat_mlps:
+            self._dense_finish.finish(sgd=False)
         ts = [m.flat_g for m in self._flat_mlps] if self._flat_mlps else \
             [q.grad for q in self._dense_params if q.grad is not None]
         return [dist.all_reduce(t, async_op=True) for t in ts]
+
+    def _unit_grad(self, loss):
+        g = getattr(self, "_unit_grad_t", None)
+        if g is None or g.device != loss.device or g.dtype != loss.dtype or g.shape != loss.shape:
+            g = self._unit_grad_t = torch.ones_like(loss)
+        return g
 
     def _dense_step(self, skip: bool = False, reduced=None):
         frozen = getattr(self, "_dense_frozen", False) or skip
@@ -1546,10 +1555,13 @@
             for w in reduced:
                 w.wait()
         if self._flat_mlps:
-            if frozen:
+            one = self.world == 1 and not frozen
+            if reduced is None:
+                self._dense_finish.finish(one, self._lr, 1.0 / self.solver.scaler)
+            if frozen or one:
                 return
             for m in self._flat_mlps:
-                if self.world > 1 and reduced is None:
+                if reduced is None:
                     _all_reduce(m.flat_g)
                 m.sgd_step(self._lr, 1.0 / self.solver.scaler)
             return
diff --git a/include/hugectr_amd.h b/include/hugectr_amd.h
--- a/include/hugectr_amd.h
+++ b/include/hugectr_amd.h
@@ -366,6 +366,34 @@
 int hctr_skinny_fc_bwd(size_t batch, int k, int n, const float* x, const void* dy, const void* y,
                        float* dw, float* db, float* workspace, int dtype, hctr_stream_t stream);
 
+int hctr_relu_bwd_bias_partials(size_t rows, int n, const void* dy, const void* y, void* dz,
+                                float* workspace, int dtype, hctr_stream_t stream);
+int hctr_logit_head_blocks(size_t batch, int k);
+int hctr_logit_head_partials(size_t batch, int k, const void* x, const void* w, const void* bias,
+                             const float* label, float grad_scale, void* dx, float* workspace,
+                             int dtype, hctr_stream_t stream);
+int hctr_skinny_fc_bwd_blocks(size_t batch, int k, int n, const void* dy, const void* y);
+int hctr_skinny_fc_bwd_partials(size_t batch, int k, int n, const float* x, const void* dy,
+                                const void* y, float* workspace, int dtype, hctr_stream_t stream);
+
+enum {
+  HCTR_DENSE_SEG_SUM_GROUPS = 0,
+  HCTR_DENSE_SEG_COLSUM = 1,
+  HCTR_DENSE_SEG_LOGIT_HEAD = 2,
+  HCTR_DENSE_SEG_SKINNY = 3,
+  HCTR_DENSE_SEG_DIRECT = 4
+};
+typedef struct {
+  int64_t kind, src, count, n, k, block0;
+  int64_t g, w, w16, dst, dst2;
+  int64_t bf16;
+  int64_t src_bf16;
+  int64_t reserved[3];
+} hctr_dense_seg;
+int hctr_dense_seg_blocks(int kind, size_t n);
+int hctr_dense_grad_finish(const hctr_dense_seg* segs, int nseg, size_t nblocks, int sgd, float lr,
+                           float grad_scale, float* loss, hctr_stream_t stream);
+
 int hctr_gemm_nt16(size_t m, int n, int k, const void* a, int lda, const void* bt, int ldb, void* c,
                    int ldc, int epilogue, const void* bias, const void* x0, const void* xl,
                    void* h_out, int dtype, hctr_stream_t stream);
```

Result: faster. 31.29 million samples/s, median of 6 (+2.8%).
